# pangenome/impg

Measured on AMD Instinct MI355X. Metric: projected ranges/sec, 1M-PAF 100k-BED -x depth 3; CPU coitrees baseline, higher is better.
Workload: dtype int32

## Files before the change

### impg_amd/csrc/capi.cpp

```cpp
#include <sys/stat.h>
#include <unistd.h>

#include <atomic>
#include <cerrno>
#include <functional>
#include <thread>
#include <chrono>
#include <cmath>
#include <cstdlib>
#include <memory>
#include <new>

#include "engine.hpp"
#include "partition.hpp"
#include "refine.hpp"

namespace impg {
thread_local std::string g_error;
void set_error(const std::string &msg) { g_error = msg; }
void render_paf(const impg_gpu_results &res, const impg_gpu_index &ix, const char *const *range_names,
                const impg_gpu_params_t &p, int32_t merge_distance, bool bedpe, std::vector<std::string> &parts);
void render_bed(const impg_gpu_results &res, const impg_gpu_index &ix, const char *const *range_names,
                const impg_gpu_params_t &p, int32_t merge_distance, std::vector<std::string> &parts);
char *join_parts(std::vector<std::string> &parts, size_t *len);
void render_fasta(const impg_gpu_results &res, const impg_gpu_index &ix, const impg_gpu_params_t &p, int32_t merge_distance, bool reverse_complement,
                  std::vector<std::string> &parts);
}

using namespace impg;


namespace impg {
static void engine_options(impg_gpu_index &ix, Engine *e) {
  const Options &o = e->opt = ix.opt;
  e->walk_allowed = o.walk_kernel != 0 && !getenv("IMPG_NO_WALK");
  e->walk_bfs = o.walk_kernel == 2;
  e->wide_emit = WideEmit{(uint32_t)o.wide_emit_cap, (uint32_t)o.wide_emit_bins, o.lookup_stats != 0};
  e->coop_count = CoopCount{(uint32_t)o.lookup_coop_span, o.lookup_coop != 0};
  e->seg_stats = ix.seg_stats;
  e->proj_stats = ix.proj_stats;
  e->place_block_levels = &ix.place_block_levels;
  e->upd_stats = ix.upd_stats;
  e->dfs_stats = ix.dfs_stats;
  e->lk_stats = ix.lk_stats;
}
static Engine *take_or_create(impg_gpu_index &ix) {
  Engine *e = nullptr;
  if (!ix.eng_free.empty()) { e = ix.eng_free.back(); ix.eng_free.pop_back(); }
  else if ((int)ix.engines.size() < ix.max_engines) {
    ix.engines.emplace_back(new Engine(ix.device));
    e = ix.engines.back().get();
  } else return nullptr;
  engine_options(ix, e);
  return e;
}
EngineLease::EngineLease(impg_gpu_index &ix_) : ix(ix_) {
  std::unique_lock<std::mutex> lk(ix.eng_m);
  while (!(e = take_or_create(ix))) ix.eng_cv.wait(lk);
}
Engine *try_lease_engine(impg_gpu_index &ix) {
  std::unique_lock<std::mutex> lk(ix.eng_m);
  return take_or_create(ix);
}
void return_engine(impg_gpu_index &ix, Engine *e) {
  e->remote = nullptr;
  e->masked = false;
  e->subset_on = false;
  std::lock_guard<std::mutex> lk(ix.eng_m);
  ix.eng_free.push_back(e);
  ix.eng_cv.notify_one();
}
EngineLease::~EngineLease() { return_engine(ix, e); }
}

namespace impg {

void require_device(int device) {
  int n = 0;
  hipError_t e = hipGetDeviceCount(&n);
  if (e != hipSuccess || n <= 0)
    throw Error{IMPG_E_HIP, "no HIP device available (libimpg_gpu has no CPU fallback)"};
  if (device < 0 || device >= n) throw Error{IMPG_E_INVALID, "device ordinal out of range"};
}

std::unique_ptr<impg_gpu_index> make_index(const impg_gpu_record_t *records, size_t n_records, const uint32_t *ops,
                                           size_t n_ops, const int64_t *seq_len, uint32_t n_seq, int bidirectional,
                                           int order_policy, int device, uint32_t shard, uint32_t n_shards,
                                           const HostSeqIndex *seq, const std::vector<uint64_t> *file_first,
                                           const uint32_t *owner) {
  if ((!records && n_records) || (!ops && n_ops) || (!seq_len && n_seq)) throw Error{IMPG_E_INVALID, "null input array"};
  require_device(device);
  auto ix = std::make_unique<impg_gpu_index>();
  ix->device = device;
  if (seq) ix->seq = *seq;
  if (file_first) {
    if (file_first->size() < 2 || file_first->front() != 0 || file_first->back() != n_records ||
        !std::is_sorted(file_first->begin(), file_first->end()))
      throw Error{IMPG_E_INVALID, "file boundaries must start at 0, end at n_records and be ascending"};
    ix->file_first = *file_first;
  }
  build_index(*ix, records, n_records, ops, n_ops, seq_len, n_seq, bidirectional != 0, order_policy, shard, n_shards, owner);
  { EngineLease warm(*ix); }
  return ix;
}

}

namespace impg {
void assemble_results(Engine &E, const impg_gpu_range_t *h_ranges, uint32_t n, const impg_gpu_params_t &p,
                      std::vector<std::unique_ptr<LevelBufs>> &levels, DevBuf &self_dev, impg_gpu_results &res, uint64_t max_rows,
                      hipEvent_t kernels_done, const std::function<void()> &on_kernels_done) {
  hipStream_t s = E.stream;
  res.ranges.assign(h_ranges, h_ranges + n);
  res.has_cigar = p.store_cigar != 0;
  RowPlan pl;
  plan_rows(E, n, p, levels, self_dev, false, pl);
  const size_t nr = pl.n_rows;
  if (nr > max_rows && n > 1) throw SplitBatch{};
  DevBuf rows, clen, coff, cpool;
  for (DevBuf *b : {&rows, &clen, &coff, &cpool}) b->pool = &E.level_pool;
  rows.reserve(std::max<size_t>(nr * sizeof(impg_gpu_interval_t), 256));
  if (res.has_cigar) clen.reserve(std::max<size_t>(nr * 4, 256));
  scatter_rows(E, levels, pl, RowSinks{rows.as<impg_gpu_interval_t>(), nullptr, nullptr, nullptr, nullptr,
                                       res.has_cigar ? clen.as<uint32_t>() : nullptr});
// ... 440 lines not shown
  IMPG_CATCH
}

int impg_gpu_index_load(const char *path, int device, impg_gpu_index_t **out) {
  IMPG_TRY
  if (!path || !out) throw Error{IMPG_E_INVALID, "null argument"};
  require_device(device);
  auto ix = std::make_unique<impg_gpu_index>();
  ix->device = device;
  load_index(*ix, path);
  { EngineLease warm(*ix); }
  *out = ix.release();
  return IMPG_OK;
  IMPG_CATCH
}

void impg_gpu_index_destroy(impg_gpu_index_t *ix) { delete ix; }

uint32_t impg_gpu_num_seqs(const impg_gpu_index_t *ix) { return (uint32_t)ix->seq.lens.size(); }
const char *impg_gpu_seq_name(const impg_gpu_index_t *ix, uint32_t id) {
  return id < ix->seq.names.size() ? ix->seq.names[id].c_str() : nullptr;
}
int64_t impg_gpu_seq_len(const impg_gpu_index_t *ix, uint32_t id) { return id < ix->seq.lens.size() ? ix->seq.lens[id] : -1; }
int64_t impg_gpu_seq_id(const impg_gpu_index_t *ix, const char *name) {
  auto it = ix->seq.name_to_id.find(name);
  return it == ix->seq.name_to_id.end() ? -1 : (int64_t)it->second;
}
size_t impg_gpu_num_targets(const impg_gpu_index_t *ix) { return ix->n_targets; }
size_t impg_gpu_target_ids(const impg_gpu_index_t *ix, uint32_t *out, size_t cap) {
  size_t k = 0;
  for (uint32_t s = 0; s + 1 < ix->h_tgt_off.size(); s++)
    if (ix->h_tgt_off[s + 1] != ix->h_tgt_off[s]) {
      if (out && k < cap) out[k] = s;
      k++;
    }
  return k;
}
size_t impg_gpu_num_entries(const impg_gpu_index_t *ix) { return ix->n_entries; }
size_t impg_gpu_num_records(const impg_gpu_index_t *ix) { return ix->n_records; }
size_t impg_gpu_device_bytes(const impg_gpu_index_t *ix) { return ix->device_bytes; }
int impg_gpu_index_approximate(const impg_gpu_index_t *ix) {
  return ix->tp_mode ? 1 : 0;
}

uint64_t impg_gpu_host_pool_trim(uint64_t keep_bytes) { return (uint64_t)impg::pinned_trim((size_t)keep_bytes); }

static_assert(option_row("walk_members")->hi == WALK_MAX_MEMBERS && option_row("wide_emit_cap")->hi == WIDE_CAP && option_row("wide_emit_bins")->hi == WIDE_BINS && option_row("lookup_coop_span")->hi == LOOKUP_COOP_CAP,
              "the option table's limits are the kernels' capacities");

int impg_gpu_set_option(impg_gpu_index_t *ix, const char *key, int64_t value) {
  IMPG_TRY
  if (!ix || !key) throw Error{IMPG_E_INVALID, "null argument"};
  const OptionRow *row = option_row(key);
  if (!row) throw Error{IMPG_E_INVALID, std::string("unknown option ") + key};
  if (!strcmp(key, "sequence_ingest_piece_bytes") && value % 16) throw Error{IMPG_E_INVALID, row->refusal};
  if (!option_store(ix->opt, *row, value)) throw Error{IMPG_E_INVALID, row->refusal};
  if (row->member || !value) return IMPG_OK;
  if (!strcmp(key, "prewarm_result_bytes")) {
    size_t cap = 0;
    void *b = pinned_take((size_t)value, cap);
    pinned_give(b, cap);
  } else if (!ix->shard && !ix->cluster) {
    IMPG_HIP(hipSetDevice(ix->device));
    EngineLease lease(*ix);
    lease->reserve_walk_slabs(*ix, value >= 2);
  }
  return IMPG_OK;
  IMPG_CATCH
}
const char *impg_gpu_option_key(size_t i) { return i < N_OPTIONS ? OPTION_TABLE[i].key : nullptr; }

struct CounterRow { const char *key; const std::atomic<uint64_t> &(*at)(const impg_gpu_index &); bool over_ranks; };
#define CTR(key, member) {key, [](const impg_gpu_index &ix) -> const std::atomic<uint64_t> & { return ix.member; }, false}
#define CTR_RANKS(key, member) {key, [](const impg_gpu_index &ix) -> const std::atomic<uint64_t> & { return ix.member; }, true}
static const CounterRow COUNTER_TABLE[] = {
    CTR("walk_launches", walk_launches), CTR("walk_fallbacks", walk_fallbacks), CTR("walk_members", walk_last_members), CTR("walk_overflow", walk_last_overflow),
    CTR("small_batches", small_batches),
    CTR("dfs_rounds", dfs_stats[0]), CTR("visited_compactions", dfs_stats[1]),
    CTR("segment_sliced_levels", seg_stats[0]), CTR("segment_retries", seg_stats[1]), CTR("segment_library_levels", seg_stats[2]),
    CTR("project_lane_levels", proj_stats[PROJ_ARM_LANE]), CTR("project_staged_levels", proj_stats[PROJ_ARM_STAGED]),
    CTR("project_staged_rows_levels", proj_stats[PROJ_ARM_STAGED_ROWS]), CTR("project_entries_slots_levels", proj_stats[PROJ_ARM_ENTRIES_SLOTS]),
    CTR("project_entries_qs_levels", proj_stats[PROJ_ARM_ENTRIES_QS]), CTR("project_entries_rows_levels", proj_stats[PROJ_ARM_ENTRIES_ROWS]),
    CTR("project_entries_ident_levels", proj_stats[PROJ_ARM_ENTRIES_IDENT]), CTR("project_tp_levels", proj_stats[PROJ_ARM_TP]),
    CTR("place_offsets_block_levels", place_block_levels),
    CTR("update_lane_groups", upd_stats[UPD_LANE]), CTR("update_mid_groups", upd_stats[UPD_MID]), CTR("update_wave_tiny_groups", upd_stats[UPD_WAVE_TINY]),
    CTR("update_wave_small_groups", upd_stats[UPD_WAVE_SMALL]), CTR("update_wave_large_groups", upd_stats[UPD_WAVE_LARGE]),
    CTR("update_inplace_groups", upd_stats[UPD_INPLACE]), CTR("update_tiled_sort_groups", upd_stats[UPD_TILED_SORT]),
    CTR("update_lane_spill_groups", upd_stats[UPD_LANE_SPILL]),
    CTR("lookup_wide_windows", lk_stats[LK_WIDE]), CTR("lookup_wide_single", lk_stats[LK_SINGLE]), CTR("lookup_wide_grouped", lk_stats[LK_GROUPED]),
    CTR("lookup_wide_group_passes", lk_stats[LK_GROUP_PASSES]), CTR("lookup_wide_overflow", lk_stats[LK_OVERFLOW]),
    CTR("lookup_coop_waves", lk_stats[LK_COOP]), CTR("lookup_lane_waves_mixed", lk_stats[LK_MIXED]), CTR("lookup_lane_waves_span", lk_stats[LK_SPAN]),
    CTR("refine_passes", refine_stats[REFINE_PASSES]), CTR("refine_candidates", refine_stats[REFINE_CANDIDATES]),
    CTR("refine_parts", refine_stats[REFINE_PARTS]), CTR("refine_rows_to_host", refine_stats[REFINE_ROWS_TO_HOST]),
    CTR("refine_longest_group", refine_stats[REFINE_LONGEST_GROUP]),
    CTR("bed_rows", bed_stats[BED_ROWS]), CTR("bed_gap_roots", bed_stats[BED_GAP_ROOTS]), CTR("bed_runs", bed_stats[BED_RUNS]),
    CTR("bed_text_pieces", bed_stats[BED_TEXT_PIECES]), CTR("bed_text_bytes", bed_stats[BED_TEXT_BYTES]),
    CTR("bedpe_rows", bedpe_stats[BEDPE_ROWS]), CTR("bedpe_runs", bedpe_stats[BEDPE_RUNS]),
    CTR("bedpe_joins_contiguous", bedpe_stats[BEDPE_JOINS_CONTIGUOUS]), CTR("bedpe_joins_gap", bedpe_stats[BEDPE_JOINS_GAP]),
    CTR("bedpe_fused_ops", bedpe_stats[BEDPE_FUSED_OPS]), CTR("bedpe_summary_ops", bedpe_stats[BEDPE_SUMMARY_OPS]),
    CTR("bedpe_text_pieces", bedpe_stats[BEDPE_TEXT_PIECES]), CTR("bedpe_text_bytes", bedpe_stats[BEDPE_TEXT_BYTES]),
    CTR("paf_rows", paf_stats[PAF_ROWS]), CTR("paf_runs", paf_stats[PAF_RUNS]),
    CTR("paf_joins_contiguous", paf_stats[PAF_JOINS_CONTIGUOUS]), CTR("paf_joins_gap", paf_stats[PAF_JOINS_GAP]),
    CTR("paf_ops_read", paf_stats[PAF_OPS_READ]), CTR("paf_ops_printed", paf_stats[PAF_OPS_PRINTED]),
    CTR("paf_through_rows", paf_stats[PAF_THROUGH_ROWS]), CTR("paf_text_pieces", paf_stats[PAF_TEXT_PIECES]),
    CTR("paf_text_bytes", paf_stats[PAF_TEXT_BYTES]),
    CTR("fasta_rows", fasta_stats[FASTA_ROWS]), CTR("fasta_records", fasta_stats[FASTA_RECORDS]),
    CTR("fasta_text_pieces", fasta_stats[FASTA_TEXT_PIECES]), CTR("fasta_text_bytes", fasta_stats[FASTA_TEXT_BYTES]),
    CTR("fasta_store_bytes", fasta_stats[FASTA_STORE_BYTES]), CTR("fasta_store_packed", fasta_stats[FASTA_STORE_PACKED]),
    CTR("fasta_store_exception_runs", fasta_stats[FASTA_STORE_EXCEPTION_RUNS]),
    CTR("sequence_ingest_pieces", ingest_stats[0]), CTR("sequence_ingest_text_bytes", ingest_stats[1]), CTR("sequence_ingest_bases", ingest_stats[2]),
    CTR("sequence_ingest_inflated_blocks", ingest_stats[3]), CTR("sequence_ingest_dropped_sequences", ingest_stats[4]),
    CTR_RANKS("build_device", build_stats[BUILD_DEVICE]), CTR_RANKS("tokenized_device", build_stats[BUILD_TOKENIZED_DEVICE]),
    CTR_RANKS("build_batches", build_stats[BUILD_BATCHES]),
};
#undef CTR
#undef CTR_RANKS
constexpr size_t N_COUNTERS = sizeof(COUNTER_TABLE) / sizeof(COUNTER_TABLE[0]);

int impg_gpu_get_counter(const impg_gpu_index_t *ix, const char *key, int64_t *value_out) {
  IMPG_TRY
  if (!ix || !key || !value_out) throw Error{IMPG_E_INVALID, "null argument"};
  for (const CounterRow &c : COUNTER_TABLE)
    if (!strcmp(c.key, key)) {
      uint64_t v = 0;
      if (c.over_ranks) for_each_rank(*ix, [&](const impg_gpu_index &r) { v += c.at(r).load(); });
      else v = c.at(*ix).load();
      *value_out = (int64_t)v;
      return IMPG_OK;
    }
  throw Error{IMPG_E_INVALID, std::string("unknown counter ") + key};
  IMPG_CATCH
}
const char *impg_gpu_counter_key(size_t i) { return i < N_COUNTERS ? COUNTER_TABLE[i].key : nullptr; }

int impg_gpu_visit_rank(uint32_t n, int order_policy, uint32_t *rank_out) {
  IMPG_TRY
  if (!rank_out && n) throw Error{IMPG_E_INVALID, "null argument"};
  if (order_policy == IMPG_ORDER_COITREES) coitrees_visit_rank(n, rank_out);
  else if (order_policy == IMPG_ORDER_SORTED) for (uint32_t i = 0; i < n; i++) rank_out[i] = i;
  else throw Error{IMPG_E_INVALID, "bad order policy"};
  return IMPG_OK;
  IMPG_CATCH
}

}
namespace impg {
void apply_mask(Engine &E, const impg_gpu_index &ix, const impg_gpu_mask_t *m, const impg_gpu_params_t &p) {
  if (!m) return;
  if (!p.transitive) throw Error{IMPG_E_INVALID, "masked_regions belong to the transitive queries"};
  const uint32_t n_seq = ix.view.n_seq;
  if (m->n_seqs && (!m->seq_id || !m->sequence_length || !m->range_off)) throw Error{IMPG_E_INVALID, "null mask array"};
  const uint64_t total = m->n_seqs ? m->range_off[m->n_seqs] : 0;
  if (total >= 0xFFFFFFF0ull) throw Error{IMPG_E_UNSUPPORTED, "mask exceeds 2^32 ranges"};
  if (total && !m->ranges) throw Error{IMPG_E_INVALID, "null mask array"};
  std::vector<uint32_t> off(n_seq + 1, 0);
  std::vector<int32_t> init_len(n_seq, 0), touch_len(n_seq, 0);
  bool has_empty = false;
  if (p.multi_impg) for (uint32_t s = 0; s < n_seq; s++) touch_len[s] = (int32_t)std::min<int64_t>(std::max<int64_t>(ix.seq.lens[s], 0), INT32_MAX);
  for (uint32_t i = 0; i < m->n_seqs; i++) {
    const uint32_t s = m->seq_id[i];
    if (s >= n_seq) throw Error{IMPG_E_INVALID, "mask names an unknown sequence id"};
    if (i && s <= m->seq_id[i - 1]) throw Error{IMPG_E_INVALID, "mask sequence ids must be strictly ascending"};
    if (m->range_off[i + 1] < m->range_off[i]) throw Error{IMPG_E_INVALID, "mask offsets must not decrease"};
    off[s + 1] = (uint32_t)(m->range_off[i + 1] - m->range_off[i]);
    init_len[s] = touch_len[s] = m->sequence_length[i];
    for (uint64_t k = m->range_off[i]; k < m->range_off[i + 1]; k++) {
      const int32_t a = m->ranges[2 * k], b = m->ranges[2 * k + 1];
// ... 841 lines not shown
```

### impg_amd/csrc/engine.cpp

```cpp
#include <cmath>
#include <cstdio>
#include <cstdlib>
#include <memory>

#include "engine.hpp"

namespace impg {

namespace {
inline unsigned bits_for(uint64_t n) {
  unsigned b = 0;
  while ((1ull << b) < n) b++;
  return b;
}
}

Engine::Engine(int device) {
  IMPG_HIP(hipSetDevice(device));
  IMPG_HIP(hipStreamCreateWithFlags(&stream, hipStreamNonBlocking));
  for (DevBuf *b : {&ord_offsets, &ord_rows}) b->pool = &level_pool;
  win_se.pool = &level_pool;
  counters.reserve(128);
  acc_slots.reserve(COUNT_BYTES);
  act_slots.reserve(COUNT_BYTES);
// ... 490 lines not shown
    }
    L.slice_pool.reserve(std::max<size_t>(L.slice_total * 4, 256));
    launch_slice_write(v, pair_entry.as<uint32_t>(), h, sl, L.n_pairs, L.slice_pos.as<uint32_t>(), L.slice_pool.as<uint32_t>(), stream);
  } else {
    L.slice_total = 0;
  }
  timed.push_back({e0, e1, 0});
  timed.push_back({e1, e2, 1});
  if (st) {
    st->pairs += P;
    st->frontier_ranges += n_fr;
    if (P) st->project_launches += 1;
  }
  return P;
}

void Engine::post_expand(const FrontierRec *fr, uint32_t n_fr, LevelBufs &L, const uint32_t *d_pair_off, uint32_t *tie_idx,
                         const uint32_t *tie_rank, SliceArrays sl) {
  HitArrays h{L.qid.as<uint32_t>(), L.coords.as<int4>()};
  if (subset_on)
    launch_subset_filter(fr, L.pair_range.as<uint32_t>(), L.n_pairs, h.qid, subset_keep.as<uint8_t>(), cur_ranges, stream);
  if (multi && L.n_pairs) {
    const size_t b = std::max<size_t>((size_t)L.n_pairs * 4, 256);
    m_dest.reserve(b); m_qid.reserve(b); m_coords.reserve(4 * b); m_pe.reserve(b);
    launch_sort5(fr, n_fr, d_pair_off, L.n_pairs, h, tie_idx, tie_rank, m_dest.as<uint32_t>(), stream);
    HitArrays h2{m_qid.as<uint32_t>(), m_coords.as<int4>()};
    SliceArrays sl2{nullptr, nullptr, nullptr, nullptr};
    if (sl.a) {
      m_sa.reserve(b); m_sn.reserve(b); m_so.reserve(b); m_sr.reserve(b);
      sl2 = SliceArrays{m_sa.as<uint32_t>(), m_sn.as<uint32_t>(), m_so.as<int32_t>(), m_sr.as<int32_t>()};
    }
    launch_permute_slots(m_dest.as<uint32_t>(), L.n_pairs, h, h2, tie_idx, m_pe.as<uint32_t>(), sl, sl2, stream);
    L.qid.swap(m_qid); L.coords.swap(m_coords);
    if (tie_idx == pair_entry.as<uint32_t>()) pair_entry.swap(m_pe);
    if (sl.a) { L.sl_a.swap(m_sa); L.sl_n.swap(m_sn); L.sl_off.swap(m_so); L.sl_rem.swap(m_sr); }
  }
}

void Engine::ordered_level(const FrontierRec *fr, uint32_t n_fr, LevelBufs &L, bool counts_by_range, uint64_t P) {
  const uint64_t total = scan(counts_by_range ? cnt.as<uint32_t>() : ord_cnt.as<uint32_t>(), L.slot_ref.as<uint32_t>(), n_fr);
  if (total != P) throw Error{IMPG_E_INVALID, "internal: a level's slot counts disagree between its two orders"};
  L.lvbase.reserve(std::max<size_t>((size_t)ord_n * 4, 256));
  launch_ord_level_bases(fr, n_fr, L.slot_ref.as<uint32_t>(), (uint32_t)P, ord_n, ord_acc.as<uint32_t>(), L.lvbase.as<uint32_t>(), stream);
}
void Engine::ordered_offsets() {
  if (ord_offsets_done) return;
  ord_offsets.reserve(((size_t)ord_n + 1) * 4);
  ord_total = scan(ord_acc.as<uint32_t>(), ord_offsets.as<uint32_t>(), ord_n + 1u);
  if (ord_total >= 0xFFFFFFF0ull) { if (split_ok) throw SplitBatch{}; throw Error{IMPG_E_UNSUPPORTED, "more than 2^32 result rows in one chunk: use smaller chunks (chunk_ranges)"}; }
  ord_rows.reserve(std::max<size_t>(ord_total * sizeof(impg_gpu_interval_t), 256));
  ord_offsets_done = true;
}
void Engine::ordered_finish(std::vector<std::unique_ptr<LevelBufs>> &levels) {
  hipEvent_t p0 = event(), p1 = event();
  IMPG_HIP(hipEventRecord(p0, stream));
  ordered_offsets();
  launch_ord_self_rows(ord_self, ord_ranges, ord_n, ord_offsets.as<uint32_t>(), ord_rows.as<impg_gpu_interval_t>(), stream);
  for (auto &Lp : levels) {
    LevelBufs &L = *Lp;
    if (L.placed || !L.n_pairs) continue;
    L.run_start.reserve(std::max<size_t>((size_t)L.n_frontier * 4, 256));
    launch_ord_run_heads(L.pair_range.as<uint32_t>(), L.n_pairs, L.run_start.as<uint32_t>(), stream);
    HitArrays h{L.qid.as<uint32_t>(), L.coords.as<int4>()};
    launch_ord_level_rows(L.frontier.as<FrontierRec>(), L.pair_range.as<uint32_t>(), L.n_pairs, h, L.run_start.as<uint32_t>(), L.slot_ref.as<uint32_t>(),
                          ord_offsets.as<uint32_t>(), L.lvbase.as<uint32_t>(), ord_min_len, ord_rows.as<impg_gpu_interval_t>(), stream);
    L.placed = true;
  }
  IMPG_HIP(hipEventRecord(p1, stream));
  IMPG_HIP(hipStreamSynchronize(stream));
  float ms = 0;
  IMPG_HIP(hipEventElapsedTime(&ms, p0, p1));
  ms_place = ms;
}

HopResult Engine::hop(const DeviceIndexView &v, const FrontierRec *fr, uint32_t n_fr, bool transitive, LevelBufs &L,
                      impg_gpu_stats_t *st, bool need_hits, bool need_rows, bool alive) {
  if (remote) return remote->hop(*this, v, fr, n_fr, transitive, L, st, need_hits, need_rows, alive);
  if (!alive) { L.n_pairs = 0; return HopResult{0, true}; }
  if (!n_fr) { L.n_pairs = 0; return HopResult{0, false}; }
  return HopResult{expand(v, fr, n_fr, transitive, L, st), false};
}

uint32_t Engine::update(const DeviceIndexView &v, const FrontierRec *fr, LevelBufs &L, uint32_t n_queries,
                        const impg_gpu_params_t &p, DevBuf &next_frontier) {
  hipEvent_t e0 = event(), e1 = event();
  IMPG_HIP(hipEventRecord(e0, stream));
  const uint32_t P = L.n_pairs;
  uint32_t n_next = 0;
  HitArrays h{L.qid.as<uint32_t>(), L.coords.as<int4>()};
  if (P) {
    const uint32_t P_slots = P;
    const bool want_flags = opt.filter_covered != 0;
    svals.reserve((size_t)P * 8);
    uint32_t seg_active = 0, seg_groups = 0;
    uint32_t *sg_run_start = nullptr, *sg_run_end = nullptr, *sg_q = nullptr, *sg_bins = nullptr;
    uint32_t seg_parts = opt.segment_groups && !want_flags && !multi && seg_group_fits(v.n_seq) && L.n_frontier > 0 ? seg_group_parts(P, n_queries, v.n_seq) : 0u;
    if (opt.segment_parts && seg_parts) {
      seg_parts = std::max(1u, std::min((uint32_t)opt.segment_parts, 4096u));
      while (seg_parts > 1 && ((uint64_t)n_queries * seg_parts >= (1ull << 31) || seg_group_bins_bytes(n_queries, v.n_seq, seg_parts) > (1ull << 30))) seg_parts >>= 1;
    }
    bool by_segments = seg_parts != 0;
    if (by_segments) {
      const uint32_t n_fr = L.n_frontier;
      seg_run.reserve(std::max<size_t>((size_t)n_fr * 8, 256));
      seg_q.reserve(std::max<size_t>((size_t)n_queries * 24 + 256, 512));
      sg_run_start = seg_run.as<uint32_t>(); sg_run_end = sg_run_start + n_fr;
      sg_q = seg_q.as<uint32_t>();
      uint32_t *qfirst = sg_q, *qlast = qfirst + n_queries, *qact = qlast + n_queries, *qdst = qact + n_queries, *qgrp = qdst + n_queries,
               *gdst = qgrp + n_queries, *unsorted = gdst + n_queries;
      const bool own_offsets = !remote && !store_cigar && L.n_frontier == expand_n_fr;
      launch_seg_bounds(fr, n_fr, n_queries, L.pair_range.as<uint32_t>(), P, sg_run_start, sg_run_end, qfirst, qlast, unsorted, stream,
                        own_offsets && last_by_place ? lo_perm.as<uint32_t>() : nullptr, own_offsets ? pair_off.as<uint32_t>() : nullptr,
                        own_offsets ? cnt.as<uint32_t>() : nullptr);
      for (int attempt = 0; attempt < 2 && by_segments; attempt++) {
        const size_t bb = seg_group_bins_bytes(n_queries, v.n_seq, seg_parts);
        sg_bins = nullptr;
        if (seg_parts > 1 || bb <= (512ull << 20)) { seg_bins.reserve(std::max<size_t>(bb, 256)); sg_bins = seg_bins.as<uint32_t>(); }
        if (seg_parts > 1) seg_tot.reserve(std::max<size_t>(seg_group_bins_bytes(n_queries, v.n_seq, 1), 256));
        launch_seg_group(true, fr, qfirst, qlast, sg_run_start, sg_run_end, h, n_queries, v.n_seq, qact, qdst, qgrp, gdst, nullptr, nullptr, nullptr, sg_bins,
                         stream, seg_parts, seg_tot.as<uint32_t>());
        uint64_t ta = 0, tg = 0;
        uint32_t bad[2] = {0, 0};
        scan2(qact, qdst, qgrp, gdst, n_queries, ta, tg, unsorted, bad, 2);
        seg_active = (uint32_t)ta;
        if (bad[0]) by_segments = false;
        else if (bad[1]) {
          const uint32_t again = seg_parts == 1 && attempt == 0 ? seg_group_parts(P, n_queries, v.n_seq, bad[1]) : 0u;
          if (again > 1) { seg_parts = again; IMPG_HIP(hipMemsetAsync(unsorted, 0, 8, stream)); if (seg_stats) seg_stats[1]++; }
          else by_segments = false;
        } else { seg_groups = (uint32_t)tg; break; }
      }
      if (by_segments && seg_parts > 1 && seg_stats) seg_stats[0]++;
    }
    if (!by_segments) {
      if (seg_stats) seg_stats[2]++;
      keys.reserve((size_t)P * 8); skeys.reserve((size_t)P * 8); vals.reserve((size_t)P * 8);
      IMPG_HIP(hipMemsetAsync(act_slots.p, 0, COUNT_BYTES, stream));
      launch_update_keys(fr, L.pair_range.as<uint32_t>(), P, h, keys.as<unsigned long long>(), vals.as<unsigned long long>(),
                         act_slots.as<unsigned long long>(), stream);
      size_t tb = sort_u64v_scratch_bytes(P);
      sort_tmp.reserve(tb);
      const unsigned sbits = std::max(1u, bits_for(v.n_seq)), qbits = std::max(1u, bits_for(n_queries));
      launch_sort_u64v(sort_tmp.p, tb, keys.as<unsigned long long>(), skeys.as<unsigned long long>(), vals.as<unsigned long long>(),
                       svals.as<unsigned long long>(), P, stream, sbits, 0);
      launch_sort_u64v(sort_tmp.p, tb, skeys.as<unsigned long long>(), keys.as<unsigned long long>(), svals.as<unsigned long long>(),
                       vals.as<unsigned long long>(), P, stream, std::min(64u, 32 + qbits + 1), 32);
      keys.swap(skeys);
      vals.swap(svals);
    }
    const uint32_t P = by_segments ? seg_active : P_slots;
    uint32_t n_groups;
    if (by_segments) n_groups = seg_groups;
    else if (want_flags) {
      head.reserve((size_t)P * 4); gid.reserve((size_t)P * 4);
      launch_group_heads(skeys.as<unsigned long long>(), P, head.as<uint32_t>(), stream);
      n_groups = (uint32_t)scan(head.as<uint32_t>(), gid.as<uint32_t>(), P);
    } else {
      const uint32_t nt = group_tiles(P);
      head.reserve((size_t)nt * 4); gid.reserve((size_t)nt * 4);
      launch_group_count(skeys.as<unsigned long long>(), P, head.as<uint32_t>(), stream);
      n_groups = (uint32_t)scan(head.as<uint32_t>(), gid.as<uint32_t>(), nt);
    }
    if (n_groups) {
      auto vt = std::make_unique<VisitedStore>(&table_pool);
      vt->keys.reserve((size_t)n_groups * 8);
      gstart.reserve((size_t)n_groups * 4);
      if (by_segments) {
        uint32_t *qfirst = sg_q, *qlast = qfirst + n_queries, *qact = qlast + n_queries, *qdst = qact + n_queries, *qgrp = qdst + n_queries,
                 *gdst = qgrp + n_queries;
        launch_seg_group(false, fr, qfirst, qlast, sg_run_start, sg_run_end, h, n_queries, v.n_seq, qact, qdst, qgrp, gdst, gstart.as<uint32_t>(),
                         vt->keys.as<unsigned long long>(), svals.as<unsigned long long>(), sg_bins, stream, seg_parts, seg_tot.as<uint32_t>());
      } else if (want_flags)
        launch_group_scatter(skeys.as<unsigned long long>(), P, head.as<uint32_t>(), gid.as<uint32_t>(), gstart.as<uint32_t>(),
                             vt->keys.as<unsigned long long>(), stream);
      else
        launch_group_fill(skeys.as<unsigned long long>(), P, gid.as<uint32_t>(), gstart.as<uint32_t>(), vt->keys.as<unsigned long long>(), stream);
      const uint32_t n_active = by_segments ? seg_active : (uint32_t)read_slots(act_slots);
      glen.reserve((size_t)n_groups * 4); old_src.reserve((size_t)n_groups * 8);
      cap.reserve((size_t)n_groups * 4); pcap.reserve((size_t)n_groups * 4);
      VisitedTables tabs = tables_view();
      launch_group_prepare(tabs, vt->keys.as<unsigned long long>(), gstart.as<uint32_t>(), n_groups, n_active,
                           glen.as<uint32_t>(), old_src.as<const int2 *>(), cap.as<uint32_t>(),
                           pcap.as<uint32_t>(), stream);
      if (getenv("IMPG_DEBUG_GROUPS")) {
        std::vector<uint32_t> hc(n_groups), hp(n_groups), hl(n_groups);
        IMPG_HIP(hipStreamSynchronize(stream));
        IMPG_HIP(hipMemcpy(hc.data(), cap.p, (size_t)n_groups * 4, hipMemcpyDeviceToHost));
        IMPG_HIP(hipMemcpy(hp.data(), pcap.p, (size_t)n_groups * 4, hipMemcpyDeviceToHost));
        IMPG_HIP(hipMemcpy(hl.data(), glen.p, (size_t)n_groups * 4, hipMemcpyDeviceToHost));
        uint64_t b[8] = {0}, hits[8] = {0};
        const uint32_t edge[8] = {16, 64, 512, 1024, 2048, 4096, 16384, 0xFFFFFFFFu};
        uint32_t mx = 0, mxl = 0;
        for (uint32_t g2 = 0; g2 < n_groups; g2++) {
          int k = 0;
          while (hc[g2] > edge[k]) k++;
          b[k]++; hits[k] += hl[g2];
          mx = std::max(mx, hc[g2]); mxl = std::max(mxl, hl[g2]);
        }
        {
          uint64_t bc[21] = {0}, bh[21] = {0};
          for (uint32_t g2 = 0; g2 < n_groups; g2++) { bc[std::min(hc[g2], 20u)]++; bh[std::min(hl[g2], 20u)]++; }
          fprintf(stderr, "[groups] by cap 1..20+:");
          for (int k2 = 1; k2 <= 20; k2++) fprintf(stderr, " %llu", (unsigned long long)bc[k2]);
          fprintf(stderr, "\n[groups] by hits 1..20+:");
          for (int k2 = 1; k2 <= 20; k2++) fprintf(stderr, " %llu", (unsigned long long)bh[k2]);
          fprintf(stderr, "\n");
        }
        fprintf(stderr, "[groups] n=%u P=%u maxcap=%u maxhits=%u | cap<=16:%llu(%llu) 64:%llu(%llu) 512:%llu(%llu) 1k:%llu(%llu) 2k:%llu(%llu) 4k:%llu(%llu) 16k:%llu(%llu) more:%llu(%llu)\n",
                n_groups, P, mx, mxl, (unsigned long long)b[0], (unsigned long long)hits[0], (unsigned long long)b[1], (unsigned long long)hits[1],
                (unsigned long long)b[2], (unsigned long long)hits[2], (unsigned long long)b[3], (unsigned long long)hits[3],
                (unsigned long long)b[4], (unsigned long long)hits[4], (unsigned long long)b[5], (unsigned long long)hits[5],
                (unsigned long long)b[6], (unsigned long long)hits[6], (unsigned long long)b[7], (unsigned long long)hits[7]);
      }
      const unsigned long long *replay_vals = svals.as<unsigned long long>();
      const bool filter = opt.filter_covered == 1 || (opt.filter_covered == 2 && tables.size() >= 2 && (uint64_t)n_active >= 8ull * n_groups);
      if (filter && n_active) {
        uint32_t *keep = keys.as<uint32_t>(), *kpos = keep + P;
        launch_covered_flags(svals.as<unsigned long long>(), head.as<uint32_t>(), gid.as<uint32_t>(), vt->keys.as<unsigned long long>(),
                             old_src.as<const int2 *>(), cap.as<uint32_t>(), glen.as<uint32_t>(), masked ? mask_touch_len.as<int32_t>() : v.seq_len,
                             n_active, keep, stream);
        const uint32_t n_kept = (uint32_t)scan(keep, kpos, n_active);
        launch_covered_compact(svals.as<unsigned long long>(), keep, kpos, n_active, vals.as<unsigned long long>(), n_kept, n_groups,
                               gstart.as<uint32_t>(), glen.as<uint32_t>(), cap.as<uint32_t>(), pcap.as<uint32_t>(), stream);
        replay_vals = vals.as<unsigned long long>();
        covered_dropped += n_active - n_kept;
      }
      vt->off.reserve((size_t)n_groups * 4);
      poff.reserve((size_t)n_groups * 4);
      uint64_t cap_total = 0, pcap_total = 0;
      big_list.reserve((size_t)n_groups * 12);
      uint32_t *d_nbig = (uint32_t *)(counters.as<uint64_t>() + 8);
      uint32_t h_lists[VU_LIST_WORDS] = {0};
      launch_big_groups(cap.as<uint32_t>(), pcap.as<uint32_t>(), n_groups, big_list.as<uint32_t>(), d_nbig, stream);
      scan2(cap.as<uint32_t>(), vt->off.as<uint32_t>(), pcap.as<uint32_t>(), poff.as<uint32_t>(), n_groups, cap_total, pcap_total, d_nbig, h_lists,
            VU_LIST_WORDS);
      if (cap_total >= 0xFFFFFFF0ull || pcap_total >= 0xFFFFFFF0ull)
        { if (split_ok) throw SplitBatch{}; throw Error{IMPG_E_UNSUPPORTED, "visited sets exceed 2^32 ranges"}; }
      vt->ranges.reserve(std::max<size_t>(cap_total * 8, 256));
      vt->len.reserve((size_t)n_groups * 4);
      pieces.reserve(std::max<size_t>(pcap_total * 8, 256));
      n_pieces.reserve((size_t)n_groups * 4);
      foff.reserve((size_t)n_groups * 4);
      launch_visited_update(replay_vals, masked ? mask_touch_len.as<int32_t>() : v.seq_len, vt->keys.as<unsigned long long>(),
                            gstart.as<uint32_t>(), glen.as<uint32_t>(), old_src.as<const int2 *>(),
                            vt->off.as<uint32_t>(), poff.as<uint32_t>(), n_groups, p.min_transitive_len,
                            p.min_distance_between_ranges, vt->ranges.as<int2>(), vt->len.as<uint32_t>(),
                            pieces.as<int2>(), n_pieces.as<uint32_t>(), cap.as<uint32_t>(), pcap.as<uint32_t>(), big_list.as<uint32_t>(),
                            d_nbig, opt.update_stats && upd_stats, stream, h_lists);
      uint64_t nn = scan(n_pieces.as<uint32_t>(), foff.as<uint32_t>(), n_groups);
      if (opt.update_stats && upd_stats && n_groups) {
        IMPG_HIP(hipMemcpyAsync(h_counters, counters.as<uint64_t>() + 8, VU_NBIG_WORDS * 4, hipMemcpyDeviceToHost, stream));
        IMPG_HIP(hipStreamSynchronize(stream));
        const uint32_t *w = reinterpret_cast<const uint32_t *>(h_counters), *reach = w + VU_REACH_BASE;
        upd_stats[UPD_LANE] += n_groups - (w[0] + w[1] + w[2] + w[6]);
        upd_stats[UPD_MID] += w[6];
        upd_stats[UPD_WAVE_TINY] += w[2];
        upd_stats[UPD_WAVE_SMALL] += w[0];
        upd_stats[UPD_WAVE_LARGE] += w[1];
        upd_stats[UPD_INPLACE] += reach[VU_REACH_INPLACE];
        upd_stats[UPD_TILED_SORT] += reach[VU_REACH_TILED_SORT];
        upd_stats[UPD_LANE_SPILL] += reach[VU_REACH_LANE_SPILL];
      }
      if (nn >= 0xFFFFFFF0ull) { if (split_ok) throw SplitBatch{}; throw Error{IMPG_E_UNSUPPORTED, "frontier exceeds 2^32 ranges"}; }
      n_next = (uint32_t)nn;
      next_frontier.reserve(std::max<size_t>((size_t)n_next * sizeof(FrontierRec), 256));
      const bool keys_too = !remote && opt.locality_min && n_next >= opt.locality_min;
      if (keys_too) { lo_key.reserve((size_t)n_next * 4); lo_idx.reserve((size_t)n_next * 4); }
      launch_frontier_emit(vt->keys.as<unsigned long long>(), poff.as<uint32_t>(), n_pieces.as<uint32_t>(),
                           foff.as<uint32_t>(), n_groups, pieces.as<int2>(), next_frontier.as<FrontierRec>(), stream,
                           keys_too ? &v : nullptr, lo_key.as<uint32_t>(), lib_sort_selected() ? lo_idx.as<uint32_t>() : nullptr);
      keys_for = keys_too ? next_frontier.p : nullptr;
      keys_n = n_next;
      vt->n_groups = n_groups;
      index_table(*vt);
      tables.push_back(std::move(vt));
      if (tables.size() + 2 >= (size_t)MAX_VISITED_TABLES) compact_tables();
    }
  }
  IMPG_HIP(hipEventRecord(e1, stream));
  timed.push_back({e0, e1, 2});
  return n_next;
}

void Engine::index_table(VisitedStore &t) {
  t.qoff.reserve(((size_t)table_queries + 1) * 4);
  launch_table_qoff(t.keys.as<unsigned long long>(), t.n_groups, table_queries, t.qoff.as<uint32_t>(), stream);
}

VisitedTables Engine::tables_view() const {
  VisitedTables t;
  memset(&t, 0, sizeof t);
  t.n_tables = (uint32_t)tables.size();
  for (size_t i = 0; i < tables.size(); i++) {
    t.t[i].keys = tables[i]->keys.as<unsigned long long>();
    t.t[i].off = tables[i]->off.as<uint32_t>();
    t.t[i].len = tables[i]->len.as<uint32_t>();
    t.t[i].ranges = tables[i]->ranges.as<int2>();
    t.t[i].qoff = tables[i]->qoff.as<uint32_t>();
    t.t[i].n_groups = tables[i]->n_groups;
  }
  if (masked) {
    t.mask_off = mask_off.as<uint32_t>();
    t.mask_ranges = mask_ranges.as<int2>();
  }
  return t;
}

uint32_t Engine::begin_transitive(const DeviceIndexView &v, const impg_gpu_range_t *d_ranges, uint32_t n,
                                  const impg_gpu_params_t &p, FrontierRec *d_self, DevBuf &frontier_out) {
  tables.clear();
  auto t = std::make_unique<VisitedStore>(&table_pool);
  t->keys.reserve((size_t)n * 8); t->off.reserve((size_t)n * 4); t->len.reserve((size_t)n * 4);
  t->ranges.reserve((size_t)n * 8);
  t->n_groups = n;
  head.reserve((size_t)n * 4); gid.reserve((size_t)n * 4);
  launch_visited_init(d_ranges, n, v.seq_len, v.n_seq, p.min_transitive_len, t->keys.as<unsigned long long>(),
                      t->off.as<uint32_t>(), t->len.as<uint32_t>(), t->ranges.as<int2>(), d_self, head.as<uint32_t>(), stream);
  uint32_t n_fr = (uint32_t)scan(head.as<uint32_t>(), gid.as<uint32_t>(), n);
  frontier_out.reserve(std::max<size_t>((size_t)n_fr * sizeof(FrontierRec), 256));
  launch_compact_frontier(d_self, head.as<uint32_t>(), gid.as<uint32_t>(), n, frontier_out.as<FrontierRec>(), stream);
  table_queries = n;
  index_table(*t);
  tables.push_back(std::move(t));
  return n_fr;
}

uint32_t Engine::begin_transitive_masked(const DeviceIndexView &v, const impg_gpu_range_t *d_ranges, uint32_t n,
                                         const impg_gpu_params_t &p, DevBuf &self, DevBuf &frontier_out) {
  tables.clear();
  auto t = std::make_unique<VisitedStore>(&table_pool);
  t->keys.reserve((size_t)n * 8); t->off.reserve((size_t)n * 4 + 4); t->len.reserve((size_t)n * 4);
  t->n_groups = n;
  cap.reserve((size_t)n * 4);
  launch_mask_caps(d_ranges, n, mask_off.as<uint32_t>(), v.n_seq, cap.as<uint32_t>(), stream);
  const uint64_t total = scan(cap.as<uint32_t>(), t->off.as<uint32_t>(), n);
  if (total >= 0xFFFFFFF0ull) { if (split_ok) throw SplitBatch{}; throw Error{IMPG_E_UNSUPPORTED, "visited sets exceed 2^32 ranges"}; }
  t->ranges.reserve(std::max<size_t>(total * 8, 256));
  pieces.reserve(std::max<size_t>(total * 8, 256));
  n_pieces.reserve((size_t)n * 4); head.reserve((size_t)n * 4); gid.reserve((size_t)n * 4);
  self_off.reserve((size_t)n * 4 + 4);
  launch_visited_init_masked(d_ranges, n, mask_init_len.as<int32_t>(), v.n_seq, mask_off.as<uint32_t>(), mask_ranges.as<int2>(),
                             p.min_transitive_len, t->off.as<uint32_t>(), t->keys.as<unsigned long long>(),
                             t->len.as<uint32_t>(), t->ranges.as<int2>(), pieces.as<int2>(), n_pieces.as<uint32_t>(),
                             head.as<uint32_t>(), stream);
  n_self = scan(n_pieces.as<uint32_t>(), self_off.as<uint32_t>(), n);
  const uint32_t n_fr = (uint32_t)scan(head.as<uint32_t>(), gid.as<uint32_t>(), n);
  self.reserve(std::max<size_t>((size_t)n_self * sizeof(FrontierRec), 256));
  frontier_out.reserve(std::max<size_t>((size_t)n_fr * sizeof(FrontierRec), 256));
  launch_masked_self_emit(d_ranges, n, t->off.as<uint32_t>(), n_pieces.as<uint32_t>(), self_off.as<uint32_t>(),
                          gid.as<uint32_t>(), p.min_transitive_len, pieces.as<int2>(), self.as<FrontierRec>(),
                          frontier_out.as<FrontierRec>(), stream);
  table_queries = n;
  index_table(*t);
  tables.push_back(std::move(t));
  return n_fr;
}

void Engine::check_params(const impg_gpu_params_t &p) {
  if (p.transitive && p.max_depth > 65535) throw Error{IMPG_E_INVALID, "max_depth is a u16 in the reference"};
// ... 36 lines not shown
  hipEvent_t t0 = event(), t1 = event();
  IMPG_HIP(hipEventRecord(t0, stream));
  if (st) memset(st, 0, sizeof *st);
  const bool transitive = p.transitive != 0;
  if (!keep && !self_out && walk_applicable(ix, n, p)) {
    ev_next = 0;
    if (run_walk(ix, d_ranges, n, p, d_count, d_cksum, st, nullptr)) return;
    if (d_count) IMPG_HIP(hipMemsetAsync(d_count, 0, (size_t)n * 8, stream));
    if (d_cksum) IMPG_HIP(hipMemsetAsync(d_cksum, 0, (size_t)n * 8, stream));
    ev_next = 0;
    timed.clear();
    IMPG_HIP(hipMemsetAsync(counters.p, 0, 64, stream));
    IMPG_HIP(hipMemsetAsync(acc_slots.p, 0, COUNT_BYTES, stream));
    t0 = event(); t1 = event();
    IMPG_HIP(hipEventRecord(t0, stream));
    if (st) memset(st, 0, sizeof *st);
  }
  if (transitive && (p.dfs || multi)) {
    ev_next = 0;
    run_dfs(ix, spec);
    return;
  }

  DevBuf *cur = &frontier_a, *nxt = &frontier_b;
  uint32_t n_fr = 0;
  cur->reserve(std::max<size_t>((size_t)n * sizeof(FrontierRec), 256));
  if (!n) {
  } else if (!transitive) {
    launch_ranges_to_frontier(d_ranges, n, cur->as<FrontierRec>(), (uint32_t *)(counters.as<uint64_t>() + 5), stream);
    n_fr = n;
  } else {
    DevBuf &self = self_out ? *self_out : self_scratch;
    self.reserve(std::max<size_t>((size_t)n * sizeof(FrontierRec), 256));
    n_fr = masked ? begin_transitive_masked(v, d_ranges, n, p, self, *cur)
                  : begin_transitive(v, d_ranges, n, p, self.as<FrontierRec>(), *cur);
    ord_self = self.as<FrontierRec>();
  }
  if (ordered_rows) {
    if (!keep || masked || multi || store_cigar || remote) throw Error{IMPG_E_INVALID, "internal: ordered rows are placed for plain and BFS batches of one GPU"};
    ord_n = n;
    ord_ranges = d_ranges;
    if (!transitive) ord_self = nullptr;
    ord_min_len = transitive ? p.min_output_length : -1;
    ord_offsets_done = false;
    ord_total = 0;
    ms_place = 0;
    ord_acc.reserve(((size_t)n + 1) * 4);
    IMPG_HIP(hipMemsetAsync(ord_acc.p, 0, ((size_t)n + 1) * 4, stream));
    launch_ord_self_count(ord_self, d_ranges, n, ord_acc.as<uint32_t>(), stream);
  }

  uint32_t depth = 0;
  for (;;) {
    const bool alive = n_fr > 0 && (!transitive || p.max_depth == 0 || depth < p.max_depth);
    const bool last = !transitive || (p.max_depth > 0 && depth + 1 >= p.max_depth);
    std::unique_ptr<LevelBufs> own;
    LevelBufs *L = &level_scratch;
    if (keep) {
      own = std::make_unique<LevelBufs>(remote_rows ? remote_rows->pool : &level_pool);
      L = own.get();
    }
    const bool want_stats = d_count || d_cksum;
    const bool owners_keep = keep && remote && remote_rows && last;
    if (owners_keep) remote_rows->level = depth;
    fuse_final = opt.fuse_final_level && last && (!keep || spec.keep_any_order || ordered_rows) && !remote;
    if (want_stats && (uint64_t)n_fr > 8192ull * n) fuse_final = false;
    fuse_need_ranges = want_stats || subset_on || keep != nullptr;
    fuse_range_places = keep != nullptr && !want_stats && !subset_on;
    if (ordered_rows) fuse_need_ranges = fuse_range_places = false;
    const HopResult hr = hop(v, cur->as<FrontierRec>(), alive ? n_fr : 0, transitive, *L, st,
                             !owners_keep && (keep || want_stats || !last), !owners_keep && (keep || d_cksum), alive);
    fuse_final = false;
    if (hr.all_dead) break;
    uint32_t n_next = 0;
    if (alive) {
      L->n_frontier = n_fr;
      if (want_stats) {
        HitArrays h{L->qid.as<uint32_t>(), L->coords.as<int4>()};
        rstat.reserve(std::max<size_t>((size_t)n_fr * 16, 256));
        launch_hit_stats(cur->as<FrontierRec>(), n_fr, L->pair_range.as<uint32_t>(), L->n_pairs, h,
                         transitive ? p.min_output_length : -1, false, rstat.as<unsigned long long>(), d_count, d_cksum, stream);
      }
      if (st) st->levels += 1;
      if (!last) n_next = update(v, cur->as<FrontierRec>(), *L, n, p, *nxt);
      if (keep && !owners_keep) {
        if (L->placed) {
        } else if (last_range_places && !remote) {
          L->frontier.adopt(win_se);
        } else {
          L->frontier.reserve(std::max<size_t>((size_t)n_fr * sizeof(FrontierRec), 256));
          IMPG_HIP(hipMemcpyAsync(L->frontier.p, cur->p, (size_t)n_fr * sizeof(FrontierRec), hipMemcpyDeviceToDevice, stream));
        }
        keep->push_back(std::move(own));
      }
    }
    if (last) break;
    std::swap(cur, nxt);
    n_fr = n_next;
    depth += 1;
  }
  if (ordered_rows) ordered_finish(*keep);
  finish_run(st, t0, t1);
}

void Engine::finish_run(impg_gpu_stats_t *st, hipEvent_t t0, hipEvent_t t1) {
  IMPG_HIP(hipEventRecord(t1, stream));
  IMPG_HIP(hipStreamSynchronize(stream));
  uint64_t hc[6];
  IMPG_HIP(hipMemcpy(hc, counters.p, 48, hipMemcpyDeviceToHost));
  if (hc[5]) throw Error{IMPG_E_INVALID, "query range must satisfy start < end"};
  if (hc[2] & 2) throw Error{IMPG_E_INVALID, "Projection resulted in negative query coordinates"};
  if (hc[2] & 4) throw Error{IMPG_E_INVALID, "CIGAR operation length exceeds 29 bits"};
  if (hc[2]) throw Error{IMPG_E_INVALID, "an alignment hit by the query has no CIGAR (missing cg:Z tag)"};
  hc[1] = read_slots(acc_slots);
  if (st) {
    st->projected = hc[1];
    float ms = 0;
    IMPG_HIP(hipEventElapsedTime(&ms, t0, t1));
    st->ms_total = ms;
    for (auto &te : timed) {
      IMPG_HIP(hipEventElapsedTime(&ms, te.a, te.b));
      if (te.kind == 0) st->ms_lookup += ms;
      else if (te.kind == 1) st->ms_project += ms;
      else st->ms_update += ms;
    }
  }
  last_projected = hc[1];
}

void Engine::compact_tables() {
  if (tables.size() < 2) return;
  uint64_t G = 0;
  for (auto &t : tables) G += t->n_groups;
  if (G >= 0xFFFFFFF0ull) throw Error{IMPG_E_UNSUPPORTED, "visited tables exceed 2^32 groups"};
  const uint32_t g = (uint32_t)G;
  VisitedTables tv = tables_view();
  d_ckey.reserve((size_t)g * 8); d_ckey2.reserve((size_t)g * 8); d_src.reserve((size_t)g * 8); d_src2.reserve((size_t)g * 8);
  uint32_t off = 0;
  for (size_t t = 0; t < tables.size(); t++) {
    launch_compact_fill(tables[t]->keys.as<unsigned long long>(), tables[t]->n_groups, (uint32_t)t,
                        d_ckey.as<unsigned long long>() + off, d_src.as<unsigned long long>() + off, stream);
    off += tables[t]->n_groups;
  }
  size_t tb = sort_u64v_scratch_bytes(g);
  sort_tmp.reserve(tb);
  launch_sort_u64v(sort_tmp.p, tb, d_ckey.as<unsigned long long>(), d_ckey2.as<unsigned long long>(),
                   d_src.as<unsigned long long>(), d_src2.as<unsigned long long>(), g, stream);
  d_flag2.reserve((size_t)g * 4); d_pos2.reserve((size_t)g * 4);
  launch_compact_last(d_ckey2.as<unsigned long long>(), g, d_flag2.as<uint32_t>(), stream);
  const uint32_t g2 = (uint32_t)scan(d_flag2.as<uint32_t>(), d_pos2.as<uint32_t>(), g);
  auto nt = std::make_unique<VisitedStore>(&table_pool);
  nt->keys.reserve((size_t)g2 * 8); nt->off.reserve((size_t)g2 * 4); nt->len.reserve((size_t)g2 * 4);
  launch_compact_select(tv, d_ckey2.as<unsigned long long>(), d_src2.as<unsigned long long>(), g, d_flag2.as<uint32_t>(),
                        d_pos2.as<uint32_t>(), nt->keys.as<unsigned long long>(), d_src.as<unsigned long long>(),
                        nt->len.as<uint32_t>(), stream);
  const uint64_t total = scan(nt->len.as<uint32_t>(), nt->off.as<uint32_t>(), g2);
  if (total >= 0xFFFFFFF0ull) throw Error{IMPG_E_UNSUPPORTED, "visited sets exceed 2^32 ranges"};
  nt->ranges.reserve(std::max<size_t>(total * 8, 256));
  launch_compact_copy(tv, d_src.as<unsigned long long>(), nt->off.as<uint32_t>(), nt->len.as<uint32_t>(), g2,
                      nt->ranges.as<int2>(), stream);
  nt->n_groups = g2;
  index_table(*nt);
  IMPG_HIP(hipStreamSynchronize(stream));
  tables.clear();
  tables.push_back(std::move(nt));
  if (dfs_stats) dfs_stats[1]++;
}
// ... 129 lines not shown
```

### impg_amd/csrc/engine.hpp

```cpp
#pragma once
#include <atomic>
#include <functional>
#include <memory>
#include <string>
#include <vector>

#include "kernels.hpp"

namespace impg {

struct LevelBufs {
  DevBuf frontier, pair_range, qid, coords;
  DevBuf sl_a, sl_n, sl_off, sl_rem, slice_pos, slice_pool;
  uint64_t slice_total = 0;
  uint32_t n_frontier = 0, n_pairs = 0;
  DevBuf slot_ref, lvbase, run_start;
  bool qs_interleaved = false;
  bool placed = false;
  LevelBufs() = default;
  explicit LevelBufs(BufPool *pool) {
    for (DevBuf *b : {&frontier, &pair_range, &qid, &coords, &sl_a, &sl_n, &sl_off, &sl_rem, &slice_pos, &slice_pool, &slot_ref, &lvbase, &run_start}) b->pool = pool;
  }
};
struct VisitedStore {
// ... 37 lines not shown
  RunSpec(const impg_gpu_range_t *d_ranges_, uint32_t n_, const impg_gpu_params_t &p_) : d_ranges(d_ranges_), n(n_), p(p_) {}
};

struct Engine {
  BufPool table_pool;
  BufPool level_pool;
  hipStream_t stream = nullptr;
  DevBuf counters;
  DevBuf acc_slots, act_slots;
  uint64_t *h_slots = nullptr;
  uint64_t read_slots(DevBuf &b);
  uint64_t *h_counters = nullptr;
  std::vector<hipEvent_t> ev_pool;
  size_t ev_next = 0;
  struct Timed { hipEvent_t a, b; int kind; };
  std::vector<Timed> timed;
  DevBuf big_list;
  DevBuf cnt, win, pair_off, pair_entry, scan_tmp, scan_tmp2, keys, skeys, vals, svals, sort_tmp, head, gid, gstart, glen, old_src,
      cap, pcap, poff, pieces, n_pieces, foff, frontier_a, frontier_b, self_scratch, ranges_dev, stat_count,
      stat_cksum, stage_off;
  LevelBufs level_scratch;
  std::vector<std::unique_ptr<VisitedStore>> tables;
  uint32_t table_queries = 0;
  void index_table(VisitedStore &t);
  uint64_t last_projected = 0;
  Options opt;
  bool split_ok = false;
  double min_identity = __builtin_nan("");
  bool store_cigar = false;
  bool multi = false;
  bool free_slot_order = false;
  bool fuse_final = false, fuse_need_ranges = false, fuse_range_places = false;
  bool last_range_places = false;
  DevBuf ord_acc, ord_offsets, ord_rows, ord_dest, ord_vpos, ord_cnt;
  uint64_t ord_total = 0;
  bool ord_offsets_done = false;
  uint32_t ord_n = 0;
  int32_t ord_min_len = -1;
  const FrontierRec *ord_self = nullptr;
  const impg_gpu_range_t *ord_ranges = nullptr;
  void ordered_level(const FrontierRec *fr, uint32_t n_fr, LevelBufs &L, bool counts_by_range, uint64_t P);
  void ordered_offsets();
  void ordered_finish(std::vector<std::unique_ptr<LevelBufs>> &levels);
  float ms_place = 0;
  DevBuf ent_work, ent_alloc;
  DevBuf win_se, tile_first;
  DevBuf place_local, place_sum, place_base;
  uint64_t covered_dropped = 0;
  DevBuf m_dest, m_qid, m_coords, m_pe, m_sa, m_sn, m_so, m_sr;
  DevBuf wide_n, wide_list;
  WideEmit wide_emit;
  CoopCount coop_count;
  std::atomic<uint64_t> *lk_stats = nullptr;
  void count_wide_paths(const DeviceIndexView &v, uint32_t n);
  DevBuf lo_key, lo_key2, lo_idx, lo_perm, lo_cnt, lo_off, lo_offp, slot_of;
  const uint32_t *stage_perm = nullptr;
  uint32_t stage_n = 0;

  explicit Engine(int device);
  ~Engine();
  hipEvent_t event();
  uint64_t read_counter(int k);
  uint64_t scan(const uint32_t *in, uint32_t *out, uint32_t n, const uint32_t *d_extra = nullptr, uint32_t *h_extra = nullptr, uint32_t n_extra = 0);
  void scan2(const uint32_t *in_a, uint32_t *out_a, const uint32_t *in_b, uint32_t *out_b, uint32_t n, uint64_t &total_a, uint64_t &total_b,
             const uint32_t *d_extra = nullptr, uint32_t *h_extra = nullptr, uint32_t n_extra = 0);
  struct RecordBlocks { const uint32_t *d_bounds; uint32_t n_blocks; };
  const uint32_t *lookup_order(const DeviceIndexView &v, const FrontierRec *fr, uint32_t n_fr, const RecordBlocks *blocks = nullptr);
  void projection_offsets(const uint32_t *d_perm, uint32_t n_fr, const uint32_t *d_cnt, uint64_t P, const uint32_t *&d_offp,
                          ProjList &pl);
  DevBuf proj_range, proj_entry;
  uint64_t expand(const DeviceIndexView &v, const FrontierRec *fr, uint32_t n_fr, bool transitive, LevelBufs &L,
                  impg_gpu_stats_t *st, bool raw = false, const RecordBlocks *blocks = nullptr);
  const void *keys_for = nullptr;
  uint32_t keys_n = 0;
  uint32_t expand_n_fr = 0;
  bool last_by_place = false;
  void post_expand(const FrontierRec *fr, uint32_t n_fr, LevelBufs &L, const uint32_t *d_pair_off, uint32_t *tie_idx,
                   const uint32_t *tie_rank, SliceArrays sl);
  Expander *remote = nullptr;
  const RunModes &modes() const { return run_modes; }
  HopResult hop(const DeviceIndexView &v, const FrontierRec *fr, uint32_t n_fr, bool transitive, LevelBufs &L,
                impg_gpu_stats_t *st, bool need_hits, bool need_rows, bool alive);
  uint32_t update(const DeviceIndexView &v, const FrontierRec *fr, LevelBufs &L, uint32_t n_queries,
                  const impg_gpu_params_t &p, DevBuf &next_frontier);
  VisitedTables tables_view() const;
  void compact_tables();
  DevBuf dk_a, dk_b, ds_a, ds_b, de_a, de_b, dd_a, dd_b, d_flag2, d_pos2, d_popdepth, d_popsel, d_perm, d_perm2, d_k32, d_k32b,
      d_src, d_src2, d_ckey, d_ckey2;
  void run_dfs(const impg_gpu_index &ix, const RunSpec &spec);
  void finish_run(impg_gpu_stats_t *st, hipEvent_t t0, hipEvent_t t1);
  static void check_params(const impg_gpu_params_t &p);
  uint32_t begin_transitive(const DeviceIndexView &v, const impg_gpu_range_t *d_ranges, uint32_t n,
                            const impg_gpu_params_t &p, FrontierRec *d_self, DevBuf &frontier_out);
  DevBuf subset_keep;
  bool subset_on = false;
  const impg_gpu_range_t *cur_ranges = nullptr;
  bool masked = false;
  DevBuf mask_off, mask_ranges, mask_init_len, mask_touch_len;
  bool mask_has_empty = false;
  uint64_t mask_ranges_total = 0, mask_lists = 0;
  DevBuf self_off;
  uint64_t n_self = 0;
  uint32_t begin_transitive_masked(const DeviceIndexView &v, const impg_gpu_range_t *d_ranges, uint32_t n,
                                   const impg_gpu_params_t &p, DevBuf &self, DevBuf &frontier_out);
  float stage_ms[3] = {0, 0, 0};
  uint64_t stage_launches = 0;
  DevBuf stage_next;
  uint32_t stage_next_n = 0, stage_queries = 0;
  void run(const impg_gpu_index &ix, const RunSpec &spec);
  static constexpr uint32_t SMALL_RANGES = 64, SMALL_PAIRS = 1u << 18;
  bool run_small(const impg_gpu_index &ix, const impg_gpu_range_t *h_ranges, uint32_t n, const impg_gpu_params_t &p,
                 impg_gpu_results &res);
  struct WalkRows {
    DevBuf rows, base, cap, n_rows;
    std::vector<uint32_t> h_n_rows;
    std::vector<unsigned long long> h_base;
  };
  bool walk_allowed = true, walk_bfs = false;
  bool walk_applicable(const impg_gpu_index &ix, uint32_t n, const impg_gpu_params_t &p) const;
  static void walk_caps(bool wide, WalkArgs &a);
  static uint64_t walk_workgroups(const impg_gpu_index &ix, bool wide);
  void reserve_walk_slabs(const impg_gpu_index &ix, bool dfs_too);
  bool run_walk(const impg_gpu_index &ix, const impg_gpu_range_t *d_ranges, uint32_t n, const impg_gpu_params_t &p,
                unsigned long long *d_count, unsigned long long *d_cksum, impg_gpu_stats_t *st, WalkRows *rows, uint32_t *h_n_rows = nullptr);
  DevBuf walk_slabs, walk_ctr, walk_ctl;
  DevBuf rstat;
  DevBuf seg_run, seg_q, seg_bins, seg_tot;
  std::atomic<uint64_t> *seg_stats = nullptr;
  std::atomic<uint64_t> *proj_stats = nullptr;
  std::atomic<uint64_t> *upd_stats = nullptr;
  std::atomic<uint64_t> *dfs_stats = nullptr;
  std::atomic<uint64_t> *place_block_levels = nullptr;
  void count_arm(int arm) { if (proj_stats && arm >= 0 && arm < PROJ_ARMS) proj_stats[arm]++; }
  uint32_t walk_group_size(const impg_gpu_index &ix, uint32_t n, const impg_gpu_params_t &p) const;
  char *small_in = nullptr;
  char *small_out = nullptr;
  void *small_out_dev = nullptr;
  size_t small_out_cap = 0;

 private:
  RunModes run_modes;
};

void build_index(impg_gpu_index &ix, const impg_gpu_record_t *records, size_t n_records, const uint32_t *cigar_ops,
                 size_t n_ops, const int64_t *seq_len, uint32_t n_seq, bool bidirectional, int order_policy,
                 uint32_t shard, uint32_t n_shards, const uint32_t *owner, const TpInput *tp = nullptr,
                 const EntryPlan *plan = nullptr);

struct EngineLease {
  impg_gpu_index &ix;
  Engine *e = nullptr;
  explicit EngineLease(impg_gpu_index &ix);
  ~EngineLease();
  EngineLease(const EngineLease &) = delete;
  Engine &operator*() { return *e; }
  Engine *operator->() { return e; }
};

#define IMPG_TRY try {
#define IMPG_CATCH                                          \
  }                                                         \
  catch (const impg::Error &e) {                            \
    impg::set_error(e.msg);                                 \
    return e.code;                                          \
  }                                                         \
  catch (const std::bad_alloc &) {                          \
    impg::set_error("host out of memory");                  \
    return IMPG_E_OOM;                                      \
  }                                                         \
  catch (const std::exception &e) {                         \
    impg::set_error(std::string("internal: ") + e.what());  \
    return IMPG_E_INVALID;                                  \
  }
void require_device(int device);
std::unique_ptr<impg_gpu_index> make_index(const impg_gpu_record_t *records, size_t n_records, const uint32_t *ops,
                                           size_t n_ops, const int64_t *seq_len, uint32_t n_seq, int bidirectional,
                                           int order_policy, int device, uint32_t shard, uint32_t n_shards,
                                           const HostSeqIndex *seq, const std::vector<uint64_t> *file_first,
                                           const uint32_t *owner);
void assemble_results(Engine &E, const impg_gpu_range_t *h_ranges, uint32_t n, const impg_gpu_params_t &p,
                      std::vector<std::unique_ptr<LevelBufs>> &levels, DevBuf &self_dev, impg_gpu_results &res,
                      uint64_t max_rows = ~0ull, hipEvent_t kernels_done = nullptr,
                      const std::function<void()> &on_kernels_done = nullptr);
const impg_gpu_range_t *upload_ranges(DevBuf &dst, const impg_gpu_range_t *ranges, size_t n, const hipStream_t *async_on);
inline void add_stats(impg_gpu_stats_t &tot, const impg_gpu_stats_t &st) {
  tot.projected += st.projected; tot.pairs += st.pairs; tot.frontier_ranges += st.frontier_ranges;
  tot.levels = std::max(tot.levels, st.levels);
  tot.ms_total += st.ms_total; tot.ms_lookup += st.ms_lookup; tot.ms_project += st.ms_project; tot.ms_update += st.ms_update;
  tot.project_launches += st.project_launches;
  tot.ms_exchange += st.ms_exchange;
}
struct StatSinks {
  unsigned long long *count = nullptr, *cksum = nullptr;
  StatSinks(DevBuf &cnt, DevBuf &ck, bool want_count, bool want_cksum, size_t n, const hipStream_t *async_on);
  void aim(RunSpec &rs, size_t b) const { rs.d_count = count ? count + b : nullptr; rs.d_cksum = cksum ? cksum + b : nullptr; }
  void home(uint64_t *per_range_count, uint64_t *per_range_checksum, size_t n) const;
};
inline std::unique_lock<std::mutex> take_turn(std::mutex *gpu_turn) {
  return gpu_turn ? std::unique_lock<std::mutex>(*gpu_turn) : std::unique_lock<std::mutex>();
}
bool run_chunk_rows(const impg_gpu_index &ix, Engine &E, const impg_gpu_range_t *d_ranges, const impg_gpu_range_t *h_ranges, size_t b,
                    size_t e, const impg_gpu_params_t &p, impg_gpu_results &part, std::mutex *gpu_turn = nullptr,
                    uint64_t max_rows = ~0ull, hipEvent_t kernels_done = nullptr,
                    const std::function<void()> &on_kernels_done = nullptr);
enum TextFormat { TEXT_BED = 0, TEXT_BEDPE = 1, TEXT_PAF = 2, TEXT_FASTA = 3, TEXT_FASTA_RC = 4 };
bool run_chunk_bed(const impg_gpu_index &ix, Engine &E, const impg_gpu_range_t *d_ranges, const impg_gpu_range_t *h_ranges,
                   const char *const *range_names, size_t b, size_t e, const impg_gpu_params_t &p, int32_t merge_distance,
                   const std::function<void(const char *, size_t)> &sink, double *seconds3, std::mutex *gpu_turn = nullptr,
                   TextFormat format = TEXT_BED);
struct RowPlan {
  DevBuf flag, pos;
  DevBuf rec_start, rec_dest;
  DevBuf offsets;
  uint64_t n_slots = 0, n_recs = 0;
  uint32_t n_rows = 0, n_self = 0;
// ... 101 lines not shown
```

### impg_amd/csrc/impg_internal.hpp

```cpp
#pragma once
#include <atomic>
#include <chrono>
#include <exception>
#include <functional>
#include <vector>
#include <hip/hip_runtime.h>

#include <algorithm>
#include <condition_variable>
#include <cstdlib>
#include <new>
#include <cstdint>
#include <cstring>
#include <memory>
#include <mutex>
#include <string>
#include <unordered_map>
#include <vector>

#include "../../include/impg_gpu.h"
#include "options.hpp"

namespace impg {

// ... 272 lines not shown
    return off;
  }
  s += name;
  return 0;
}

enum BuildStat { BUILD_DEVICE, BUILD_TOKENIZED_DEVICE, BUILD_BATCHES };
void for_each_rank(const impg_gpu_index &ix, const std::function<void(const impg_gpu_index &)> &f);
enum BedStat { BED_ROWS, BED_GAP_ROOTS, BED_RUNS, BED_TEXT_PIECES, BED_TEXT_BYTES };
enum BedpeStat { BEDPE_ROWS, BEDPE_RUNS, BEDPE_JOINS_CONTIGUOUS, BEDPE_JOINS_GAP, BEDPE_FUSED_OPS, BEDPE_SUMMARY_OPS, BEDPE_TEXT_PIECES, BEDPE_TEXT_BYTES };
enum PafStat { PAF_ROWS, PAF_RUNS, PAF_JOINS_CONTIGUOUS, PAF_JOINS_GAP, PAF_OPS_READ, PAF_OPS_PRINTED, PAF_THROUGH_ROWS, PAF_TEXT_PIECES, PAF_TEXT_BYTES };
size_t bed_merge(impg_gpu_interval_t *iv, size_t n, int32_t merge_distance, bool merge_strands);
void query_axis_merge(std::vector<impg_gpu_interval_t> &rows, int32_t merge_distance, bool merge_strands);

enum FastaStat { FASTA_ROWS, FASTA_RECORDS, FASTA_TEXT_PIECES, FASTA_TEXT_BYTES, FASTA_STORE_BYTES, FASTA_STORE_PACKED, FASTA_STORE_EXCEPTION_RUNS };
struct SeqStore {
  std::vector<std::string> names;
  std::vector<uint64_t> off;
  std::string bases;
  std::unordered_map<std::string, uint32_t> by_name;
  bool device_only = false;
  void add(const std::string &name, const char *b, size_t n);
};
inline const SeqStore &host_copy(const SeqStore &st) {
  if (st.device_only)
    throw Error{IMPG_E_UNSUPPORTED, "the sequences were loaded straight into HBM (impg_gpu_index_load_sequences) and have no host copy: "
                                    "attach them with impg_gpu_index_set_sequences for FASTA text written on the host"};
  return st;
}
constexpr uint32_t SEQ_ABSENT = 0xFFFFFFFFu;
constexpr uint64_t SEQ_NOT_IN_HBM = ~0ull;
constexpr size_t SEQ_PAD = 16;
struct SeqRun { uint32_t start, end; uint8_t byte; };
void seq_exception_runs(const char *bases, size_t n, std::vector<SeqRun> &runs);
struct SeqRef { const char *bases; uint64_t len; };
void fasta_range_text(std::vector<impg_gpu_interval_t> &rows, int32_t merge_distance, bool reverse_complement,
                      const std::function<bool(uint32_t, std::string &, SeqRef &)> &fetch, std::string &text);
void partition_fasta_text(const impg_gpu_partition_row_t *rows, size_t n, const std::function<bool(uint32_t, std::string &, SeqRef &)> &fetch,
                          std::string &text);

struct Engine;
struct ShardCtx;
struct Cluster;

}

struct impg_gpu_index {
  int device = 0;
  hipStream_t stream = nullptr;
  impg::HostSeqIndex seq;
  size_t n_records = 0, n_entries = 0, n_tiles = 0, n_targets = 0;
  std::vector<uint32_t> h_tgt_off;
  std::vector<uint64_t> file_first;
  impg::DevBuf d_seg, d_starts, d_ends, d_ends_t, d_pmax, d_starts_lvl, d_pmax_lvl, d_rank, d_mrank, d_entries, d_ops, d_ext_cp, d_idp, d_seq_len, d_pfx;
  impg::DeviceIndexView view{};
  static constexpr int N_BLOBS = 15;
  impg::DevBuf *blob(int k);
  size_t blob_bytes[N_BLOBS] = {};
  bool multi_file = false;
  bool tp_mode = false;
  void bind_view(uint32_t n_seq, uint32_t sorted_order);
  std::atomic<size_t> device_bytes{0};
  std::mutex idl_m;
  void ensure_identity_lines();
  std::atomic<bool> has_identity_lines{false};
  bool lacks_identity_lines() const {
    return !tp_mode && n_tiles && blob_bytes[14] && !has_identity_lines.load(std::memory_order_acquire);
  }
  std::vector<std::unique_ptr<impg::Engine>> engines;
  std::vector<impg::Engine *> eng_free;
  std::mutex eng_m;
  std::condition_variable eng_cv;
  int max_engines = 4;
  impg::Options opt;
  struct RowsPool : impg::BufPool { RowsPool() { shared = true; } } rows_pool;
  mutable std::atomic<uint64_t> walk_launches{0}, walk_fallbacks{0}, walk_last_members{1}, walk_last_overflow{0};
  mutable std::atomic<uint64_t> small_batches{0};
  mutable std::atomic<uint64_t> dfs_stats[2] = {};
  mutable std::atomic<uint64_t> build_stats[3] = {};
  mutable std::atomic<uint64_t> mask_table_uploads{0}, result_rows_to_host{0};
  mutable std::atomic<uint64_t> seg_stats[3] = {};
  mutable std::atomic<uint64_t> proj_stats[8] = {};
  mutable std::atomic<uint64_t> place_block_levels{0};
  mutable std::atomic<uint64_t> upd_stats[8] = {};
  mutable std::atomic<uint64_t> lk_stats[8] = {};
  mutable std::atomic<uint64_t> refine_stats[5] = {};
  mutable std::atomic<uint64_t> bed_stats[5] = {};
  void bed_stats_reset() const { for (auto &b : bed_stats) b = 0; }
  mutable std::atomic<uint64_t> bedpe_stats[8] = {};
  void bedpe_stats_reset() const { for (auto &b : bedpe_stats) b = 0; }
  mutable std::atomic<uint64_t> paf_stats[9] = {};
  void paf_stats_reset() const { for (auto &b : paf_stats) b = 0; }
  mutable std::atomic<uint64_t> fasta_stats[7] = {};
  mutable std::atomic<uint64_t> ingest_stats[5] = {};
  void fasta_stats_reset() const { for (int k = 0; k < impg::FASTA_STORE_BYTES; k++) fasta_stats[k] = 0; }
  std::shared_ptr<const impg::SeqStore> seq_store;
  std::vector<uint32_t> store_of_id;
  impg::DevBuf d_seq_bases, d_seq_off;
  bool seq_packed = false;
  impg::DevBuf d_seq_run_off, d_seq_runs, d_seq_run_byte, d_seq_blk_off, d_seq_blk;
  void drop_device_sequences();
  impg::ShardCtx *shard = nullptr;
  impg::Cluster *cluster = nullptr;
  impg_gpu_index();
  ~impg_gpu_index();
};

struct impg_gpu_results {
  std::vector<uint64_t> offsets;
  impg::HostArr<impg_gpu_interval_t> intervals;
  std::vector<impg_gpu_range_t> ranges;
  bool has_cigar = false;
  bool approximate = false;
  impg::HostArr<uint64_t> cigar_off;
  impg::HostArr<uint32_t> cigar_ops;
  uint64_t projected = 0;
  double run_s = 0, assemble_s = 0;
};
```

### impg_amd/csrc/kernels.hip

```cpp
#include <hip/hip_runtime.h>

#include <cstring>
#include <type_traits>

#include "device_prims.hpp"
#include "impg_internal.hpp"
#include "kernels.hpp"

namespace impg {

__device__ __forceinline__ unsigned lane_id() { return threadIdx.x & 63u; }
__device__ __forceinline__ unsigned long long lanemask_lt() { return (1ull << lane_id()) - 1ull; }

template <int CTRL, int ROW_MASK>
__device__ __forceinline__ uint32_t dpp_or0(uint32_t x) {
  return (uint32_t)__builtin_amdgcn_update_dpp(0, (int)x, CTRL, ROW_MASK, 0xF, false);
}
__device__ __forceinline__ uint32_t wave_incl_scan(uint32_t x) {
  x += dpp_or0<0x111, 0xF>(x);
  x += dpp_or0<0x112, 0xF>(x);
  x += dpp_or0<0x114, 0xF>(x);
  x += dpp_or0<0x118, 0xF>(x);
  x += dpp_or0<0x142, 0xA>(x);
  x += dpp_or0<0x143, 0xC>(x);
// ... 2953 lines not shown
  bool should_add = true;
  if (mdbr > 0) {
    const uint32_t idx = list_lower_bound(R, len, start);
    if (idx > 0 && abs(start - R.y(idx - 1)) < mdbr) should_add = false;
    if (should_add && idx < len && abs(R.x(idx) - end) < mdbr) should_add = false;
  }
  if (!should_add) return;
  if (start < 0) start = 0;
  if (end > sequence_length) end = sequence_length;
  int32_t current = start;
  const uint32_t pos = list_lower_bound(R, len, start);
  uint32_t i = pos;
  if (i > 0 && R.y(i - 1) > start) i -= 1;
  while (i < len && current < end) {
    const int32_t rx = R.x(i), ry = R.y(i);
    if (rx > end) break;
    if (current < rx) {
      if (abs(rx - current) >= min_transitive_len) emit(current, rx);
    }
    current = max(current, ry);
    i += 1;
  }
  if (current < end) {
    if (abs(end - current) >= min_transitive_len) emit(current, end);
  }
  uint32_t mfrom;
  if (pos > 0 && R.y(pos - 1) >= start) {
    R.y(pos - 1) = max(R.y(pos - 1), end);
    mfrom = pos - 1;
  } else if (pos < len && end >= R.x(pos)) {
    R.x(pos) = min(start, R.x(pos));
    R.y(pos) = max(end, R.y(pos));
    mfrom = pos;
  } else {
    grow();
    for (uint32_t k = len; k > pos; k--) { R.x(k) = R.x(k - 1); R.y(k) = R.y(k - 1); }
    R.x(pos) = start;
    R.y(pos) = end;
    len += 1;
    return;
  }
  uint32_t write = mfrom, read = mfrom + 1;
  while (read < len) {
    if (R.y(write) >= R.x(read)) {
      R.y(write) = max(R.y(write), R.y(read));
    } else {
      write += 1;
      const int32_t tx = R.x(write), ty = R.y(write);
      R.x(write) = R.x(read); R.y(write) = R.y(read);
      R.x(read) = tx; R.y(read) = ty;
    }
    read += 1;
  }
  len = write + 1;
}
template <class L>
__device__ __forceinline__ uint32_t replay_hits(const L &R, uint32_t len, const unsigned long long *__restrict__ svals,
                                                uint32_t st, uint32_t n, int32_t sequence_length,
                                                int32_t min_transitive_len, int32_t mdbr, int2 *__restrict__ P, uint32_t &np) {
  for (uint32_t t = 0; t < n; t++) {
    const unsigned long long iv = svals[st + t];
    replay_one(R, len, (int32_t)(uint32_t)(iv >> 32), (int32_t)(uint32_t)iv, sequence_length, min_transitive_len, mdbr,
               [&](int32_t a, int32_t b) { P[np++] = make_int2(a, b); }, [] {});
  }
  return len;
}
#ifdef IMPG_VU_CLOCKS
constexpr uint32_t VU_CLK_ROWS = 1024;
__device__ unsigned long long g_vu_clk[VU_CLK_ROWS][16];
#define VU_MARK(i) do { asm volatile("s_waitcnt vmcnt(0) lgkmcnt(0)" ::: "memory"); vu_t[i] = __builtin_readcyclecounter(); } while (0)
#else
#define VU_MARK(i) do { } while (0)
#endif
typedef const unsigned long long __attribute__((address_space(1))) *global_list_t;
__device__ __forceinline__ int2 list_range(global_list_t p, uint32_t i) {
  const unsigned long long v = p[i];
  return make_int2((int32_t)(uint32_t)v, (int32_t)(uint32_t)(v >> 32));
}
#ifndef IMPG_VU_WAVES
#define IMPG_VU_WAVES 6
#endif
#pragma clang diagnostic push
#pragma clang diagnostic ignored "-Wpass-failed"
template <uint32_t CAP, bool LISTED>
__global__ __launch_bounds__(64) __attribute__((amdgpu_waves_per_eu(IMPG_VU_WAVES, IMPG_VU_WAVES)))
void visited_update_kernel(const unsigned long long *__restrict__ svals,
                                                            const int32_t *__restrict__ seq_len,
                                                            const unsigned long long *__restrict__ gkey,
                                                            const uint32_t *__restrict__ gstart,
                                                            const uint32_t *__restrict__ glen,
                                                            const unsigned long long *__restrict__ old_src,
                                                            const uint32_t *__restrict__ cap,
                                                            const uint32_t *__restrict__ noff,
                                                            const uint32_t *__restrict__ poff, uint32_t n_groups,
                                                            int32_t min_transitive_len, int32_t mdbr,
                                                            int2 *__restrict__ new_ranges, uint32_t *__restrict__ new_len,
                                                            int2 *__restrict__ pieces, uint32_t *__restrict__ n_pieces,
                                                            const uint32_t *__restrict__ list, const uint32_t *__restrict__ n_list,
                                                            uint32_t *__restrict__ reach) {
  __shared__ int32_t lds_x[CAP * 64], lds_y[CAP * 64];
  const uint32_t n_items = LISTED ? *n_list : n_groups;
  for (uint32_t item0 = blockIdx.x * 64u; item0 < n_items; item0 += gridDim.x * 64u) {
  const uint32_t item = item0 + threadIdx.x;
#ifdef IMPG_VU_CLOCKS
  unsigned long long vu_t[8];
  VU_MARK(0);
#endif
  const bool have = item < n_items;
  const uint32_t g = LISTED ? list[min(item, n_items - 1u)] : item;
  const uint32_t gi = min(g, n_groups - 1u);
  const uint32_t c_ = cap[gi], n_ = glen[gi], st_ = gstart[gi], no = noff[gi], po = poff[gi];
  const global_list_t src_ = (global_list_t)old_src[gi];
  const unsigned long long key = gkey[gi];
  const uint32_t c = have ? c_ : 0u;
  const bool mine = have && (LISTED || c <= VU_TINY_MAX);
  const uint32_t n = mine ? n_ : 0u, st = mine ? st_ : 0u;
  const uint32_t olen = mine ? c - n : 0u;
  int2 *R = new_ranges + no;
  int2 *P = pieces + po;
  VU_MARK(1);
  const int32_t sequence_length = seq_len[(uint32_t)(key & 0xFFFFFFFFull)];
  const unsigned long long *hp = svals + st;
  const uint32_t hl = max(n, 1u) - 1u;
  unsigned long long h0 = hp[0], h1 = hp[min(1u, hl)], h2 = hp[min(2u, hl)], h3 = hp[min(3u, hl)];
  const global_list_t src = olen ? src_ : (global_list_t)(unsigned long long)(uintptr_t)svals;
  const uint32_t sl = max(olen, 1u) - 1u;
  const int2 s0 = list_range(src, 0), s1 = list_range(src, min(1u, sl)), s2 = list_range(src, min(2u, sl)), s3 = list_range(src, min(3u, sl));
  VU_MARK(2);
  uint32_t len = olen, np = 0;
  VU_MARK(3);
  const bool fast = mine;
  const ListInLds A{lds_x + threadIdx.x, lds_y + threadIdx.x};
  if (fast) {
    if (olen > 0) { A.x(0) = s0.x; A.y(0) = s0.y; }
    if (olen > 1) { A.x(1) = s1.x; A.y(1) = s1.y; }
    if (olen > 2) { A.x(2) = s2.x; A.y(2) = s2.y; }
    if (olen > 3) { A.x(3) = s3.x; A.y(3) = s3.y; }
    for (uint32_t i = 4; i < olen; i += 4) {
      const uint32_t l = olen - 1u;
      const int2 r0 = list_range(src, i), r1 = list_range(src, min(i + 1u, l)), r2 = list_range(src, min(i + 2u, l)), r3 = list_range(src, min(i + 3u, l));
      A.x(i) = r0.x; A.y(i) = r0.y;
      if (i + 1u < olen) { A.x(i + 1u) = r1.x; A.y(i + 1u) = r1.y; }
      if (i + 2u < olen) { A.x(i + 2u) = r2.x; A.y(i + 2u) = r2.y; }
      if (i + 3u < olen) { A.x(i + 3u) = r3.x; A.y(i + 3u) = r3.y; }
    }
  }
  VU_MARK(4);
  const uint32_t nf = fast ? n : 0u;
  const uint32_t nmax = wave_max_u32(nf);
  bool spilled = false;
  auto spill = [&]() {
    for (uint32_t k = 0; k < np; k++) P[k] = make_int2(A.x(CAP - 1u - k), A.y(CAP - 1u - k));
    spilled = true;
  };
  auto emit = [&](int32_t a, int32_t b) {
    if (!spilled && len + np >= CAP) spill();
    if (!spilled) { A.x(CAP - 1u - np) = a; A.y(CAP - 1u - np) = b; }
    else P[np] = make_int2(a, b);
    np += 1;
  };
  auto grow = [&]() { if (!spilled && len + np >= CAP) spill(); };
  for (uint32_t t0 = 0; t0 < nmax; t0 += 4u) {
    unsigned long long q0 = 0, q1 = 0, q2 = 0, q3 = 0;
    if (t0 + 4u < nmax && nf) {
      const unsigned long long *hp = svals + st;
      const uint32_t l = nf - 1u;
      q0 = hp[min(t0 + 4u, l)]; q1 = hp[min(t0 + 5u, l)]; q2 = hp[min(t0 + 6u, l)]; q3 = hp[min(t0 + 7u, l)];
    }
#pragma nounroll
    for (uint32_t k = 0; k < 4u; k++) {
      const unsigned long long iv = h0;
      h0 = h1; h1 = h2; h2 = h3;
      if (t0 + k < nf)
        replay_one(A, len, (int32_t)(uint32_t)(iv >> 32), (int32_t)(uint32_t)iv, sequence_length, min_transitive_len, mdbr, emit, grow);
    }
    h0 = q0; h1 = q1; h2 = q2; h3 = q3;
  }
  VU_MARK(5);
  if (fast) for (uint32_t i = 0; i < len; i++) R[i] = make_int2(A.x(i), A.y(i));
  VU_MARK(6);
  if (fast && !spilled) {
    const uint32_t T = CAP - 1u;
    for (uint32_t i = 1; i < np; i++) {
      const int32_t tx = A.x(T - i), ty = A.y(T - i);
      uint32_t j = i;
      while (j > 0 && A.x(T - (j - 1u)) > tx) { A.x(T - j) = A.x(T - (j - 1u)); A.y(T - j) = A.y(T - (j - 1u)); j--; }
      A.x(T - j) = tx; A.y(T - j) = ty;
    }
    if (np) {
      uint32_t w = 0;
      int32_t cx = A.x(T), cy = A.y(T);
      for (uint32_t r = 1; r < np; r++) {
        const int32_t rx = A.x(T - r), ry = A.y(T - r);
        if (cy >= rx) cy = max(cy, ry);
        else { P[w] = make_int2(cx, cy); w += 1; cx = rx; cy = ry; }
      }
      P[w] = make_int2(cx, cy);
      np = w + 1;
    }
  } else if (mine && np > 1 && np <= CAP) {
    const ListInLds S{lds_x + threadIdx.x, lds_y + threadIdx.x};
    for (uint32_t i = 0; i < np; i += 4) {
      const uint32_t l = np - 1u;
      const int2 r0 = P[i], r1 = P[min(i + 1u, l)], r2 = P[min(i + 2u, l)], r3 = P[min(i + 3u, l)];
      S.x(i) = r0.x; S.y(i) = r0.y;
      if (i + 1u < np) { S.x(i + 1u) = r1.x; S.y(i + 1u) = r1.y; }
      if (i + 2u < np) { S.x(i + 2u) = r2.x; S.y(i + 2u) = r2.y; }
      if (i + 3u < np) { S.x(i + 3u) = r3.x; S.y(i + 3u) = r3.y; }
    }
    for (uint32_t i = 1; i < np; i++) {
      const int32_t tx = S.x(i), ty = S.y(i);
      uint32_t j = i;
      while (j > 0 && S.x(j - 1) > tx) { S.x(j) = S.x(j - 1); S.y(j) = S.y(j - 1); j--; }
      S.x(j) = tx; S.y(j) = ty;
    }
    uint32_t w = 0;
    int32_t cx = S.x(0), cy = S.y(0);
    for (uint32_t r = 1; r < np; r++) {
      const int32_t rx = S.x(r), ry = S.y(r);
      if (cy >= rx) cy = max(cy, ry);
      else { P[w] = make_int2(cx, cy); w += 1; cx = rx; cy = ry; }
    }
    P[w] = make_int2(cx, cy);
    np = w + 1;
  } else if (mine) {
    for (uint32_t i = 1; i < np; i++) {
      int2 x = P[i];
      uint32_t j = i;
      while (j > 0 && P[j - 1].x > x.x) { P[j] = P[j - 1]; j--; }
      P[j] = x;
    }
    uint32_t w = 0;
    for (uint32_t r = 1; r < np; r++) {
      if (P[w].y >= P[r].x) P[w].y = max(P[w].y, P[r].y);
      else { w += 1; P[w] = P[r]; }
    }
    if (np) np = w + 1;
  }
  if (mine) {
    new_len[g] = len;
    n_pieces[g] = np;
  }
  {
    const unsigned long long sp = __ballot(fast && spilled);
    if (reach && sp && threadIdx.x == 0) atomicAdd(reach + VU_REACH_LANE_SPILL, (uint32_t)__popcll(sp));
  }
#ifdef IMPG_VU_CLOCKS
  VU_MARK(7);
  {
    const unsigned long long slow = 0ull, regp = __ballot(fast && spilled);
    const uint32_t nsum = wave_incl_scan(n), smax = 0u;
    const uint32_t ntot = (uint32_t)__builtin_amdgcn_readlane((int)nsum, 63);
    if (threadIdx.x == 0 && (blockIdx.x & 15u) == 0u) {
      unsigned long long *row = g_vu_clk[(blockIdx.x >> 4) % VU_CLK_ROWS];
      for (int i = 0; i < 7; i++) atomicAdd(&row[i], vu_t[i + 1] - vu_t[i]);
      atomicAdd(&row[8], 1ull);
      atomicAdd(&row[9], slow ? 1ull : 0ull);
      atomicAdd(&row[10], (unsigned long long)nmax);
      atomicAdd(&row[11], (unsigned long long)ntot);
      atomicAdd(&row[12], (unsigned long long)smax);
      atomicAdd(&row[13], regp ? 1ull : 0ull);
      if (slow) atomicAdd(&row[14], vu_t[3] - vu_t[2]);
    }
  }
#endif
  }
}
#pragma clang diagnostic pop
#ifdef IMPG_VU_CLOCKS
extern "C" void impg_gpu_debug_vu_clocks(unsigned long long *out) {
  static unsigned long long rows[VU_CLK_ROWS][16];
  (void)hipDeviceSynchronize();
  (void)hipMemcpyFromSymbol(rows, HIP_SYMBOL(g_vu_clk), sizeof(rows));
  for (int k = 0; k < 16; k++) { out[k] = 0; for (uint32_t r = 0; r < VU_CLK_ROWS; r++) out[k] += rows[r][k]; }
  memset(rows, 0, sizeof(rows));
  (void)hipMemcpyToSymbol(HIP_SYMBOL(g_vu_clk), rows, sizeof(rows));
}
#endif

template <class L> __device__ __forceinline__ void order_point(const L &) { __syncthreads(); }
struct ListSoA {
  int32_t *px, *py;
  __device__ __forceinline__ int32_t &x(uint32_t i) const { return px[i]; }
  __device__ __forceinline__ int32_t &y(uint32_t i) const { return py[i]; }
};
template <> __device__ __forceinline__ void order_point<ListSoA>(const ListSoA &) { __builtin_amdgcn_wave_barrier(); }
template <class L> __device__ __forceinline__ uint32_t wave_lower_bound(const L &R, uint32_t n, int32_t s) {
  uint32_t lo = 0, hi = n;
  const uint32_t lane = lane_id();
  while (hi - lo > 64u) {
    const uint32_t step = (hi - lo + 63u) >> 6;
    const uint32_t idx = lo + (lane + 1u) * step - 1u;
    const bool lt = idx < hi && R.x(idx) < s;
    const uint32_t c = (uint32_t)__popcll(__ballot(lt));
    const uint32_t nlo = lo + c * step;
    hi = min(hi, nlo + step);
    lo = nlo;
  }
  const uint32_t idx = lo + lane;
  return lo + (uint32_t)__popcll(__ballot(idx < hi && R.x(idx) < s));
}
template <class L> __device__ __forceinline__ void wave_shift_up(const L &R, uint32_t pos, uint32_t len) {
  const uint32_t lane = lane_id();
  for (uint32_t top = len; top > pos;) {
    const uint32_t base = top > pos + 64u ? top - 64u : pos;
    const uint32_t at = base + lane;
    const bool on = at < top;
    int32_t vx = 0, vy = 0;
    if (on) { vx = R.x(at); vy = R.y(at); }
    top = base;
    order_point(R);
    if (on) { R.x(at + 1) = vx; R.y(at + 1) = vy; }
    order_point(R);
  }
}
template <class L> __device__ __forceinline__ void wave_shift_down(const L &R, uint32_t from, uint32_t len, uint32_t k) {
  const uint32_t lane = lane_id();
  for (uint32_t base = from; base < len; base += 64u) {
    const uint32_t i = base + lane;
    int32_t vx = 0, vy = 0;
    if (i < len) { vx = R.x(i); vy = R.y(i); }
    order_point(R);
    if (i < len) { R.x(i - k) = vx; R.y(i - k) = vy; }
    order_point(R);
  }
}
__device__ __forceinline__ void sort_cx_lane(int2 &v, uint32_t partner) {
  int2 o;
// ... 540 lines not shown
  }
  keep[i] = covered ? 0u : 1u;
}
__global__ __launch_bounds__(256) void covered_compact_kernel(const unsigned long long *__restrict__ svals, const uint32_t *__restrict__ keep,
                                                              const uint32_t *__restrict__ kpos, uint32_t n_active,
                                                              unsigned long long *__restrict__ out) {
  const uint32_t i = blockIdx.x * 256u + threadIdx.x;
  if (i < n_active && keep[i]) out[kpos[i]] = svals[i];
}
__global__ __launch_bounds__(256) void covered_regroup_kernel(const uint32_t *__restrict__ kpos, uint32_t n_active, uint32_t n_kept,
                                                              uint32_t n_groups, uint32_t *__restrict__ gstart, uint32_t *__restrict__ glen,
                                                              uint32_t *__restrict__ cap, uint32_t *__restrict__ pcap) {
  const uint32_t g = blockIdx.x * 256u + threadIdx.x;
  if (g >= n_groups) return;
  const uint32_t st = gstart[g], n = glen[g], en = st + n;
  const uint32_t ns = kpos[st], ne = en < n_active ? kpos[en] : n_kept;
  const uint32_t olen = cap[g] - n;
  gstart[g] = ns;
  glen[g] = ne - ns;
  cap[g] = olen + (ne - ns);
  pcap[g] = olen + 2u * (ne - ns);
}

constexpr uint32_t BG_THREADS = 1024, BG_PER_THREAD = 4;
__global__ __launch_bounds__(BG_THREADS) void big_groups_kernel(const uint32_t *__restrict__ cap, const uint32_t *__restrict__ pcap,
                                                                uint32_t n_groups, uint32_t *__restrict__ big_list,
                                                                uint32_t *__restrict__ n_big) {
  __shared__ uint32_t cnt[4], base[4];
  if (threadIdx.x < 4u) cnt[threadIdx.x] = 0u;
  __syncthreads();
  uint32_t tier[BG_PER_THREAD], off[BG_PER_THREAD];
#pragma unroll
  for (uint32_t k = 0; k < BG_PER_THREAD; k++) {
    const uint32_t g = (blockIdx.x * BG_PER_THREAD + k) * BG_THREADS + threadIdx.x;
    const uint32_t c = g < n_groups ? cap[g] : 0u;
    uint32_t t = 0;
    if (c > VU_TINY_MAX) {
      if (c <= VU_MID_MAX) t = 1u;
      else {
        const uint32_t old_len = 2u * c - pcap[g];
        t = c + 64u <= VW_CAP_TINY ? 2u : (old_len + VW_SMALL_HEADROOM <= VW_CAP_SMALL - 64u ? 3u : 4u);
      }
    }
    tier[k] = t;
    off[k] = 0u;
    if (__ballot(t != 0u)) {
#pragma unroll
      for (uint32_t tt = 1; tt <= 4u; tt++) {
        const unsigned long long m = __ballot(t == tt);
        if (!m) continue;
        uint32_t o = 0;
        if (lane_id() == 0) o = atomicAdd(&cnt[tt - 1u], (uint32_t)__popcll(m));
        o = (uint32_t)__shfl((int)o, 0);
        if (t == tt) off[k] = o + (uint32_t)__popcll(m & lanemask_lt());
      }
    }
  }
  __syncthreads();
  if (threadIdx.x < 4u) {
    const uint32_t slot = threadIdx.x == 0u ? 6u : (threadIdx.x == 1u ? 2u : (threadIdx.x == 2u ? 0u : 1u));
    base[threadIdx.x] = cnt[threadIdx.x] ? atomicAdd(&n_big[slot], cnt[threadIdx.x]) : 0u;
  }
  __syncthreads();
#pragma unroll
  for (uint32_t k = 0; k < BG_PER_THREAD; k++) {
    const uint32_t g = (blockIdx.x * BG_PER_THREAD + k) * BG_THREADS + threadIdx.x;
    const uint32_t t = tier[k];
    if (!t) continue;
    const uint32_t pos = base[t - 1u] + off[k];
    if (t == 1u) big_list[2u * (size_t)n_groups + pos] = g;
    else if (t == 2u) big_list[(size_t)n_groups + pos] = g;
    else if (t == 3u) big_list[pos] = g;
    else big_list[n_groups - 1u - pos] = g;
  }
}

__global__ __launch_bounds__(256) void frontier_emit_kernel(const unsigned long long *__restrict__ gkey,
                                                            const uint32_t *__restrict__ poff,
                                                            const uint32_t *__restrict__ n_pieces,
                                                            const uint32_t *__restrict__ foff, uint32_t n_groups,
                                                            const int2 *__restrict__ pieces,
                                                            FrontierRec *__restrict__ out, const SegDesc *__restrict__ seg,
                                                            const int32_t *__restrict__ seq_len, uint32_t n_seq,
                                                            uint32_t *__restrict__ key, uint32_t *__restrict__ idx) {
  const uint32_t g = blockIdx.x * 256u + threadIdx.x;
  const bool in = g < n_groups;
  const unsigned long long k = in ? gkey[g] : 0ull;
  const uint32_t np = in ? n_pieces[g] : 0u;
  const uint32_t po = in ? poff[g] : 0u;
  const uint32_t fo = in ? foff[g] : 0xFFFFFFFFu;
  const uint32_t first = (uint32_t)__shfl((int)fo, 0);
  const unsigned long long live = __ballot(in);
  if (!live) return;
  const int last = 63 - __builtin_clzll(live);
  const uint32_t end = (uint32_t)__shfl((int)(fo + np), last);
  for (uint32_t o = first + lane_id(); o - lane_id() < end; o += 64u) {
    uint32_t j = 0;
#pragma unroll
    for (uint32_t st = 32u; st > 0u; st >>= 1) {
      const uint32_t f = (uint32_t)__shfl((int)fo, (int)(j + st));
      j += f <= o ? st : 0u;
    }
    const uint32_t fj = (uint32_t)__shfl((int)fo, (int)j), pj = (uint32_t)__shfl((int)po, (int)j);
    const uint32_t klo = (uint32_t)__shfl((int)(uint32_t)k, (int)j), khi = (uint32_t)__shfl((int)(uint32_t)(k >> 32), (int)j);
    if (o < end) {
      const int2 piece = pieces[pj + (o - fj)];
      FrontierRec f;
      f.target_id = klo;
      f.start = piece.x;
      f.end = piece.y;
      f.qidx = khi;
      out[o] = f;
      if (key) { key[o] = order_key(seg, seq_len, n_seq, klo, piece.x); if (idx) idx[o] = o; }
    }
  }
}

__global__ __launch_bounds__(256) void subset_filter_kernel(const FrontierRec *__restrict__ fr,
                                                            const uint32_t *__restrict__ pair_range, uint32_t n_pairs,
                                                            uint32_t *__restrict__ qid, const uint8_t *__restrict__ keep,
                                                            const impg_gpu_range_t *__restrict__ ranges) {
  const uint32_t p = blockIdx.x * 256u + threadIdx.x;
  if (p >= n_pairs) return;
  const uint32_t q = qid[p];
  if (q == HIT_NONE) return;
  if (keep[q]) return;
  if (q != ranges[fr[pair_range[p]].qidx].target_id) qid[p] = HIT_NONE;
}

__global__ __launch_bounds__(256) void mask_caps_kernel(const impg_gpu_range_t *__restrict__ ranges, uint32_t n,
                                                        const uint32_t *__restrict__ mask_off, uint32_t n_seq,
                                                        uint32_t *__restrict__ cap) {
  const uint32_t q = blockIdx.x * 256u + threadIdx.x;
  if (q >= n) return;
  const uint32_t t = ranges[q].target_id;
  cap[q] = (t < n_seq ? mask_off[t + 1] - mask_off[t] : 0u) + 1u;
}
__global__ __launch_bounds__(64) void visited_init_masked_kernel(const impg_gpu_range_t *__restrict__ ranges, uint32_t n,
                                                                 const int32_t *__restrict__ init_len, uint32_t n_seq,
                                                                 const uint32_t *__restrict__ mask_off,
                                                                 const int2 *__restrict__ mask_ranges,
                                                                 int32_t min_transitive_len, const uint32_t *__restrict__ loff,
                                                                 unsigned long long *__restrict__ keys,
                                                                 uint32_t *__restrict__ len_out, int2 *__restrict__ rng,
                                                                 int2 *__restrict__ pieces, uint32_t *__restrict__ n_self,
                                                                 uint32_t *__restrict__ n_front) {
  const uint32_t q = blockIdx.x * 64u + threadIdx.x;
  if (q >= n) return;
  const impg_gpu_range_t r = ranges[q];
  int32_t start = min(r.start, r.end), end = max(r.start, r.end);
  const bool known = r.target_id < n_seq;
  const int32_t sequence_length = known ? init_len[r.target_id] : 0;
  int2 *R = rng + loff[q];
  int2 *P = pieces + loff[q];
  uint32_t len = 0;
  if (known) {
    const uint32_t a = mask_off[r.target_id];
    len = mask_off[r.target_id + 1] - a;
    for (uint32_t i = 0; i < len; i++) R[i] = mask_ranges[a + i];
  }
  if (start < 0) start = 0;
  if (end > sequence_length) end = sequence_length;
  uint32_t np = 0, nf = 0;
  int32_t current = start;
  uint32_t i = lower_bound_start(R, len, start);
  if (i > 0 && R[i - 1].y > start) i -= 1;
  while (i < len && current < end) {
    const int2 rg = R[i];
    if (rg.x > end) break;
    if (current < rg.x) {
      P[np++] = make_int2(current, rg.x);
      nf += abs(rg.x - current) >= min_transitive_len;
    }
    current = max(current, rg.y);
    i += 1;
  }
  if (current < end) {
    P[np++] = make_int2(current, end);
    nf += abs(end - current) >= min_transitive_len;
  }
  const uint32_t pos = lower_bound_start(R, len, start);
  bool merge = true;
  uint32_t mfrom = 0;
  if (pos > 0 && R[pos - 1].y >= start) {
    R[pos - 1].y = max(R[pos - 1].y, end);
    mfrom = pos - 1;
  } else if (pos < len && end >= R[pos].x) {
    R[pos].x = min(start, R[pos].x);
    R[pos].y = max(end, R[pos].y);
    mfrom = pos;
  } else {
    for (uint32_t k = len; k > pos; k--) R[k] = R[k - 1];
    R[pos] = make_int2(start, end);
    len += 1;
    merge = false;
  }
// ... 757 lines not shown
  if (!n) return;
  prims::radix_sort_pairs(tmp, tmp_bytes, kin, kout, vin, vout, n, 0, end_bit, s);
}
bool seg_group_fits(uint32_t n_seq) { return n_seq <= SEG_MAX_SEQ; }
size_t seg_group_bins_bytes(uint32_t n_queries, uint32_t n_seq, uint32_t parts) {
  return (size_t)n_queries * parts * ((std::max(n_seq, 1u) + 63u) & ~63u) * 4;
}
uint32_t seg_group_parts(uint64_t n_hits, uint32_t n_queries, uint32_t n_seq, uint64_t largest_query) {
  if (!n_queries) return 1;
  const uint64_t per_query = std::max<uint64_t>(n_hits / n_queries, largest_query);
  if (per_query <= (largest_query ? SEG_BIG_QUERY : SEG_BIG_QUERY / 2)) return 1;
  const uint64_t parts = (per_query + SEG_SLICE_HITS - 1) / SEG_SLICE_HITS;
  if (parts > SEG_MAX_PARTS || (uint64_t)n_queries * parts >= (1ull << 31)) return 0;
  if (seg_group_bins_bytes(n_queries, n_seq, (uint32_t)parts) > (1ull << 30)) return 0;
  return (uint32_t)parts;
}
void launch_seg_bounds(const FrontierRec *fr, uint32_t n_fr, uint32_t n_queries, const uint32_t *pair_range, uint32_t n_pairs, uint32_t *run_start,
                       uint32_t *run_end, uint32_t *qfirst, uint32_t *qlast, uint32_t *unsorted, hipStream_t s, const uint32_t *off_perm,
                       const uint32_t *pair_off, const uint32_t *cnt) {
  IMPG_HIP(hipMemsetAsync(qfirst, 0, (size_t)n_queries * 4, s));
  IMPG_HIP(hipMemsetAsync(qlast, 0, (size_t)n_queries * 4, s));
  IMPG_HIP(hipMemsetAsync(unsorted, 0, 8, s));
  if (pair_off && cnt) {
    if (n_fr) run_bounds_by_offsets_kernel<<<cdiv(n_fr, 256), 256, 0, s>>>(off_perm, pair_off, cnt, n_fr, run_start, run_end);
  } else {
    IMPG_HIP(hipMemsetAsync(run_start, 0, (size_t)n_fr * 4, s));
    IMPG_HIP(hipMemsetAsync(run_end, 0, (size_t)n_fr * 4, s));
    if (n_pairs) run_bounds_kernel<<<cdiv(n_pairs, 256), 256, 0, s>>>(pair_range, n_pairs, run_start, run_end);
  }
  if (n_fr) query_bounds_kernel<<<cdiv(n_fr, 256), 256, 0, s>>>(fr, n_fr, n_queries, qfirst, qlast, unsorted);
}
void launch_seg_group(bool count_only, const FrontierRec *fr, const uint32_t *qfirst, const uint32_t *qlast, const uint32_t *run_start,
                      const uint32_t *run_end, HitArrays h, uint32_t n_queries, uint32_t n_seq, uint32_t *qact, const uint32_t *qdst, uint32_t *qgrp,
                      const uint32_t *gdst, uint32_t *gstart, unsigned long long *gkey, unsigned long long *svals, uint32_t *qbins, hipStream_t s,
                      uint32_t parts, uint32_t *qtot) {
  if (!n_queries) return;
  if (parts > 1u && (!qbins || !qtot)) throw Error{IMPG_E_INVALID, "internal: sliced segment grouping without its counters"};
  const uint32_t nb = (std::max(n_seq, 1u) + 63u) & ~63u;
  uint32_t nbits = 1;
  while ((1u << nbits) < n_seq) nbits++;
  const uint32_t grid = cdiv(n_queries * parts, SEG_WAVES);
  if (count_only)
    seg_group_kernel<true><<<grid, 64 * SEG_WAVES, SEG_WAVES * nb * 4, s>>>(fr, qfirst, qlast, run_start, run_end, h, n_queries, nb, nbits, qact, qdst, qgrp,
                                                                          gdst, gstart, gkey, svals, qbins, parts, qtot);
  else
    seg_group_kernel<false><<<grid, 64 * SEG_WAVES, SEG_WAVES * nb * 4, s>>>(fr, qfirst, qlast, run_start, run_end, h, n_queries, nb, nbits, qact, qdst, qgrp,
                                                                           gdst, gstart, gkey, svals, qbins, parts, qtot);
  if (count_only && parts > 1u) {
    IMPG_HIP(hipMemsetAsync(qact, 0, (size_t)n_queries * 4, s));
    IMPG_HIP(hipMemsetAsync(qgrp, 0, (size_t)n_queries * 4, s));
    seg_parts_scan_kernel<<<dim3(n_queries, cdiv(nb, 256u)), 256, 0, s>>>(qbins, nb, parts, qtot, qact, qgrp);
  }
}
uint32_t group_tiles(uint32_t n) { return (n + GROUP_TILE - 1u) / GROUP_TILE; }
void launch_group_count(const unsigned long long *skeys, uint32_t n, uint32_t *tile_heads, hipStream_t s) {
  if (n) group_count_kernel<<<group_tiles(n), 256, 0, s>>>(skeys, n, tile_heads);
}
void launch_group_fill(const unsigned long long *skeys, uint32_t n, const uint32_t *tile_base, uint32_t *gstart, unsigned long long *gkey, hipStream_t s) {
  if (n) group_fill_kernel<<<group_tiles(n), 256, 0, s>>>(skeys, n, tile_base, gstart, gkey);
}
void launch_group_heads(const unsigned long long *skeys, uint32_t n, uint32_t *head, hipStream_t s) {
  if (!n) return;
  group_heads_kernel<<<cdiv(n, 256), 256, 0, s>>>(skeys, n, head);
}
void launch_group_scatter(const unsigned long long *skeys, uint32_t n, const uint32_t *head, const uint32_t *gid,
                          uint32_t *gstart, unsigned long long *gkey, hipStream_t s) {
  if (!n) return;
  group_scatter_kernel<<<cdiv(n, 256), 256, 0, s>>>(skeys, n, head, gid, gstart, gkey);
}
void launch_table_qoff(const unsigned long long *keys, uint32_t n_groups, uint32_t n_queries, uint32_t *qoff, hipStream_t s) {
  table_qoff_kernel<<<cdiv((uint64_t)n_queries + 1, 256), 256, 0, s>>>(keys, n_groups, n_queries, qoff);
}
void launch_group_prepare(const VisitedTables &vt, const unsigned long long *gkey, const uint32_t *gstart,
                          uint32_t n_groups, uint32_t n_active, uint32_t *glen, const int2 **old_src,
                          uint32_t *cap, uint32_t *pcap, hipStream_t s) {
  if (!n_groups) return;
  group_prepare_kernel<<<cdiv(n_groups, 256), 256, 0, s>>>(vt, gkey, gstart, n_groups, n_active, glen, old_src, cap, pcap);
}
void launch_visited_update(const unsigned long long *svals, const int32_t *seq_len,
                           const unsigned long long *gkey, const uint32_t *gstart, const uint32_t *glen,
                           const int2 *const *old_src, const uint32_t *noff, const uint32_t *poff,
                           uint32_t n_groups, int32_t min_transitive_len, int32_t mdbr, int2 *new_ranges,
                           uint32_t *new_len, int2 *pieces, uint32_t *n_pieces, const uint32_t *cap, const uint32_t *pcap,
                           uint32_t *big_list, uint32_t *n_big, bool count_reach, hipStream_t s, const uint32_t *h_lists) {
  if (!n_groups) return;
  uint32_t *reach = count_reach ? n_big + VU_REACH_BASE : nullptr;
  const uint32_t n_small = h_lists[0], n_large = h_lists[1], n_tiny = h_lists[2], n_mid = h_lists[6];
  const unsigned long long *srcs = reinterpret_cast<const unsigned long long *>(old_src);
  visited_update_kernel<VU_LDS_CAP, false><<<cdiv(n_groups, 64), 64, 0, s>>>(svals, seq_len, gkey, gstart, glen, srcs, cap, noff, poff, n_groups,
                                                                             min_transitive_len, mdbr, new_ranges, new_len, pieces, n_pieces,
                                                                             nullptr, nullptr, reach);
  const uint32_t mid_blocks = std::min<uint32_t>(cdiv(n_mid, 64), 256u * std::min(32u, (160u * 1024u) / (VU_MID_CAP * 64u * 8u)));
  if (n_mid)
    visited_update_kernel<VU_MID_CAP, true><<<mid_blocks, 64, 0, s>>>(svals, seq_len, gkey, gstart, glen, srcs, cap, noff, poff, n_groups,
                                                                      min_transitive_len, mdbr, new_ranges, new_len, pieces, n_pieces,
                                                                      big_list + 2u * (size_t)n_groups, n_big + 6, reach);
  const uint32_t blocks = std::min<uint32_t>(n_small, 256u * std::min(32u, (160u * 1024u) / (VW_CAP_SMALL * 8u)));
  if (n_small)
    visited_update_wave_kernel<VW_CAP_SMALL><<<blocks, 64, 0, s>>>(
        svals, seq_len, gkey, gstart, glen, old_src, cap, noff, poff, big_list, n_big, n_big + 3, 0u, min_transitive_len, mdbr, new_ranges,
        new_len, pieces, n_pieces, reach);
  if (n_tiny)
    visited_update_wave_kernel<VW_CAP_TINY, true><<<std::min<uint32_t>(n_tiny, 256u * 32u), 64, 0, s>>>(
        svals, seq_len, gkey, gstart, glen, old_src, cap, noff, poff, big_list + n_groups, n_big + 2, n_big + 5, 0u, min_transitive_len, mdbr, new_ranges,
        new_len, pieces, n_pieces, reach);
  if (n_large)
    visited_update_wave_kernel<VW_CAP_LARGE><<<std::min<uint32_t>(n_large, 256u * 5u), 64, 0, s>>>(
        svals, seq_len, gkey, gstart, glen, old_src, cap, noff, poff, big_list, n_big + 1, n_big + 4, n_groups, min_transitive_len, mdbr,
        new_ranges, new_len, pieces, n_pieces, reach);
}
void launch_big_groups(const uint32_t *cap, const uint32_t *pcap, uint32_t n_groups, uint32_t *big_list, uint32_t *n_big, hipStream_t s) {
  if (!n_groups) return;
  (void)hipMemsetAsync(n_big, 0, VU_NBIG_WORDS * 4, s);
  big_groups_kernel<<<cdiv(n_groups, BG_THREADS * BG_PER_THREAD), BG_THREADS, 0, s>>>(cap, pcap, n_groups, big_list, n_big);
}
void launch_covered_flags(const unsigned long long *svals, const uint32_t *head, const uint32_t *gid,
                          const unsigned long long *gkey, const int2 *const *old_src, const uint32_t *cap, const uint32_t *glen,
                          const int32_t *seq_len, uint32_t n_active, uint32_t *keep, hipStream_t s) {
  if (n_active) covered_flags_kernel<<<cdiv(n_active, 256), 256, 0, s>>>(svals, head, gid, gkey, old_src, cap, glen, seq_len, n_active, keep);
}
void launch_covered_compact(const unsigned long long *svals, const uint32_t *keep, const uint32_t *kpos, uint32_t n_active,
                            unsigned long long *out, uint32_t n_kept, uint32_t n_groups, uint32_t *gstart, uint32_t *glen, uint32_t *cap,
                            uint32_t *pcap, hipStream_t s) {
  if (n_active) covered_compact_kernel<<<cdiv(n_active, 256), 256, 0, s>>>(svals, keep, kpos, n_active, out);
  if (n_groups) covered_regroup_kernel<<<cdiv(n_groups, 256), 256, 0, s>>>(kpos, n_active, n_kept, n_groups, gstart, glen, cap, pcap);
}
void launch_frontier_emit(const unsigned long long *gkey, const uint32_t *poff, const uint32_t *n_pieces,
                          const uint32_t *foff, uint32_t n_groups, const int2 *pieces, FrontierRec *out, hipStream_t s,
                          const DeviceIndexView *v, uint32_t *key, uint32_t *idx) {
  if (!n_groups) return;
  frontier_emit_kernel<<<cdiv(n_groups, 256), 256, 0, s>>>(gkey, poff, n_pieces, foff, n_groups, pieces, out, v ? v->seg : nullptr,
                                                           v ? v->seq_len : nullptr, v ? v->n_seq : 0u, v ? key : nullptr, v ? idx : nullptr);
}
void launch_subset_filter(const FrontierRec *fr, const uint32_t *pair_range, uint32_t n_pairs, uint32_t *qid,
                          const uint8_t *keep, const impg_gpu_range_t *ranges, hipStream_t s) {
  if (n_pairs) subset_filter_kernel<<<cdiv(n_pairs, 256), 256, 0, s>>>(fr, pair_range, n_pairs, qid, keep, ranges);
}
void launch_mask_caps(const impg_gpu_range_t *ranges, uint32_t n, const uint32_t *mask_off, uint32_t n_seq, uint32_t *cap,
                      hipStream_t s) {
  if (n) mask_caps_kernel<<<cdiv(n, 256), 256, 0, s>>>(ranges, n, mask_off, n_seq, cap);
}
void launch_visited_init_masked(const impg_gpu_range_t *ranges, uint32_t n, const int32_t *init_len, uint32_t n_seq,
                                const uint32_t *mask_off, const int2 *mask_ranges, int32_t min_transitive_len,
                                const uint32_t *loff, unsigned long long *keys, uint32_t *len, int2 *rng, int2 *pieces,
                                uint32_t *n_self, uint32_t *n_front, hipStream_t s) {
  if (n) visited_init_masked_kernel<<<cdiv(n, 64), 64, 0, s>>>(ranges, n, init_len, n_seq, mask_off, mask_ranges,
                                                                min_transitive_len, loff, keys, len, rng, pieces, n_self, n_front);
}
void launch_masked_self_emit(const impg_gpu_range_t *ranges, uint32_t n, const uint32_t *loff, const uint32_t *n_self,
                             const uint32_t *self_off, const uint32_t *front_off, int32_t min_transitive_len,
                             const int2 *pieces, FrontierRec *self_out, FrontierRec *frontier_out, hipStream_t s) {
  if (n) masked_self_emit_kernel<<<cdiv(n, 256), 256, 0, s>>>(ranges, n, loff, n_self, self_off, front_off, min_transitive_len,
                                                              pieces, self_out, frontier_out);
}
void launch_visited_init(const impg_gpu_range_t *ranges, uint32_t n, const int32_t *seq_len, uint32_t n_seq,
                         int32_t min_transitive_len, unsigned long long *keys, uint32_t *off, uint32_t *len, int2 *rng,
                         FrontierRec *self_iv, uint32_t *in_frontier, hipStream_t s) {
  if (!n) return;
  visited_init_kernel<<<cdiv(n, 256), 256, 0, s>>>(ranges, n, seq_len, n_seq, min_transitive_len, keys, off, len, rng, self_iv, in_frontier);
}
void launch_compact_frontier(const FrontierRec *in, const uint32_t *flag, const uint32_t *pos, uint32_t n,
                             FrontierRec *out, hipStream_t s) {
  if (!n) return;
  compact_frontier_kernel<<<cdiv(n, 256), 256, 0, s>>>(in, flag, pos, n, out);
}
void launch_ranges_to_frontier(const impg_gpu_range_t *ranges, uint32_t n, FrontierRec *out, uint32_t *bad, hipStream_t s) {
  if (!n) return;
  ranges_to_frontier_kernel<<<cdiv(n, 256), 256, 0, s>>>(ranges, n, out, bad);
}
void launch_frontier_to_stack(const FrontierRec *fr, uint32_t n, const uint32_t *pop_depth, bool use_depth,
                              unsigned long long *key, int32_t *st, int32_t *en, uint32_t *depth, hipStream_t s) {
  if (!n) return;
  frontier_to_stack_kernel<<<cdiv(n, 256), 256, 0, s>>>(fr, n, pop_depth, use_depth ? 1 : 0, key, st, en, depth);
}
void launch_dfs_pop_flags(const unsigned long long *key, const uint32_t *depth, uint32_t n, uint32_t max_depth,
                          bool pop_front, uint32_t *fr_flag, uint32_t *keep_flag, uint32_t *pop_depth, uint32_t *pop_sel, uint32_t n_queries,
                          hipStream_t s) {
  if (!n) return;
  IMPG_HIP(hipMemsetAsync(pop_sel, pop_front ? 0xFF : 0x00, (size_t)n_queries * 4, s));
  dfs_pop_select_kernel<<<cdiv(n, 256), 256, 0, s>>>(key, depth, n, max_depth, pop_front ? 1 : 0, pop_sel);
  dfs_pop_flags_kernel<<<cdiv(n, 256), 256, 0, s>>>(key, depth, n, pop_front ? 1 : 0, pop_sel, fr_flag, keep_flag, pop_depth);
}
void launch_sort5(const FrontierRec *fr, uint32_t n, const uint32_t *pair_off, uint32_t n_pairs, HitArrays h,
                  const uint32_t *pair_entry, const uint32_t *mrank, uint32_t *dest, hipStream_t s) {
  if (n && n_pairs) sort5_kernel<<<wave_grid(n), 256, 0, s>>>(fr, n, pair_off, n_pairs, h, pair_entry, mrank, dest);
}
void launch_permute_slots(const uint32_t *dest, uint32_t n_pairs, HitArrays in, HitArrays out, const uint32_t *pe_in,
                          uint32_t *pe_out, SliceArrays sin, SliceArrays sout, hipStream_t s) {
  if (n_pairs) permute_slots_kernel<<<cdiv(n_pairs, 256), 256, 0, s>>>(dest, n_pairs, in, out, pe_in, pe_out, sin, sout);
}
void launch_dfs_pop_scatter(const unsigned long long *key, const int32_t *st, const int32_t *en, const uint32_t *depth,
                            uint32_t n, const uint32_t *fr_flag, const uint32_t *fr_pos, const uint32_t *keep_flag,
                            const uint32_t *keep_pos, FrontierRec *fr_out, unsigned long long *key_out, int32_t *st_out,
                            int32_t *en_out, uint32_t *depth_out, hipStream_t s) {
  if (!n) return;
  dfs_pop_scatter_kernel<<<cdiv(n, 256), 256, 0, s>>>(key, st, en, depth, n, fr_flag, fr_pos, keep_flag, keep_pos, fr_out,
                                                     key_out, st_out, en_out, depth_out);
}
void launch_iota(uint32_t *v, uint32_t n, hipStream_t s) { if (n) iota_kernel<<<cdiv(n, 256), 256, 0, s>>>(v, n); }
void launch_gather_u32(const uint32_t *src, const uint32_t *idx, uint32_t n, uint32_t *dst, hipStream_t s) {
  if (n) gather_u32_kernel<<<cdiv(n, 256), 256, 0, s>>>(src, idx, n, dst);
}
void launch_gather_u64(const unsigned long long *src, const uint32_t *idx, uint32_t n, unsigned long long *dst, hipStream_t s) {
  if (n) gather_u64_kernel<<<cdiv(n, 256), 256, 0, s>>>(src, idx, n, dst);
}
void launch_run_heads(const unsigned long long *skeys, uint32_t n, uint32_t *head, hipStream_t s) {
  if (n) run_heads_kernel<<<cdiv(n, 256), 256, 0, s>>>(skeys, n, head);
}
void launch_run_starts(const uint32_t *head, const uint32_t *gid, uint32_t n, uint32_t *gstart, hipStream_t s) {
  if (n) run_starts_kernel<<<cdiv(n, 256), 256, 0, s>>>(head, gid, n, gstart);
}
void launch_dfs_merge(const uint32_t *gstart, uint32_t n_groups, uint32_t n, const uint32_t *perm, const int32_t *st,
                      const int32_t *en, const uint32_t *depth, int32_t *st_m, int32_t *en_m, uint32_t *depth_m,
                      uint32_t *cnt, hipStream_t s) {
  if (n_groups) dfs_merge_kernel<<<cdiv(n_groups, 64), 64, 0, s>>>(gstart, n_groups, n, perm, st, en, depth, st_m, en_m, depth_m, cnt);
// ... 279 lines not shown
```

### impg_amd/csrc/kernels.hpp

```cpp
#pragma once
#include <hip/hip_runtime.h>

#include <cstdint>

#include "impg_internal.hpp"

namespace impg {

struct FrontierRec {
  uint32_t target_id;
  int32_t start, end;
  uint32_t qidx;
};

struct HitArrays {
  uint32_t *qid;
  int4 *c;
};

struct SliceArrays {
  uint32_t *a;
  uint32_t *n;
  int32_t *off;
  int32_t *rem;
// ... 81 lines not shown
                        const uint32_t *pair_off, const uint4 *win, uint32_t *pair_range, uint32_t *pair_entry,
                        const uint32_t *perm, const uint32_t *offp, ProjList pl, const uint32_t *wide_n,
                        const uint32_t *wide_list, hipStream_t s, bool by_place = false, bool wide_only = false, WideEmit we = WideEmit{});
constexpr uint32_t ROUTE_WORLD_MAX = 1024;
void launch_route_keys(const FrontierRec *fr, uint32_t n, uint32_t world, const uint32_t *owner, uint32_t n_seq, uint32_t *key,
                       uint32_t *idx, unsigned long long *hist, hipStream_t s);
void launch_hits_pack(const FrontierRec *fr, const uint32_t *pair_range, uint32_t n_pairs, HitArrays h, const uint32_t *pair_entry,
                      const uint32_t *mrank, uint32_t words, void *out, hipStream_t s, const uint32_t *slice_n = nullptr);
void launch_hits_slice_n(const void *in, uint32_t n, uint32_t *cnt, hipStream_t s);
void launch_hits_unpack(const void *in, uint32_t n, uint32_t words, uint32_t n_front, const uint32_t *run_start, const uint32_t *off,
                        uint32_t *pair_range, HitArrays h, uint32_t *mslot, hipStream_t s, const uint32_t *slice_at = nullptr,
                        uint32_t *slice_pos = nullptr, uint32_t *slice_n = nullptr);
void launch_route_gather(const FrontierRec *fr, const uint32_t *perm, uint32_t n, FrontierRec *out, hipStream_t s);
void launch_route_gather_ranges(const FrontierRec *fr, const uint32_t *perm, uint32_t n, uint32_t range_base, FrontierRec *out, hipStream_t s);
void launch_partial_stats_add(const unsigned long long *in, uint32_t blocks, uint32_t n, unsigned long long *out, hipStream_t s);
void launch_frontier_gather(const FrontierRec *fr, const uint32_t *perm, uint32_t n, FrontierRec *out, hipStream_t s);
void launch_reorder_runs(const uint32_t *hits, uint32_t n, uint32_t words, uint32_t n_front, uint32_t *run_start,
                         uint32_t *run_len, uint32_t *err, hipStream_t s);
void launch_order_keys(const DeviceIndexView &v, const FrontierRec *fr, uint32_t n, uint32_t *key, uint32_t *idx, hipStream_t s,
                       const uint32_t *bounds = nullptr, uint32_t n_blocks = 0, uint32_t block_shift = 0);
void launch_scatter_u32(const uint32_t *in, const uint32_t *perm, uint32_t n, uint32_t *out, hipStream_t s);
enum ScanForm : int { SCAN_FORM_LOOKBACK = 0, SCAN_FORM_THREE_KERNEL = 1 };
int launch_exclusive_scan(const uint32_t *d_in, uint32_t *d_out, uint32_t n, unsigned long long *d_bsum,
                          unsigned long long *d_total, hipStream_t s);
size_t scan_scratch_bytes(uint32_t n);
void scan_tile_sizes(uint32_t *lookback_tile, uint32_t *three_kernel_tile);
enum ProjArm : int {
  PROJ_ARM_NONE = -1,
  PROJ_ARM_LANE = 0,
  PROJ_ARM_STAGED,
  PROJ_ARM_STAGED_ROWS,
  PROJ_ARM_ENTRIES_SLOTS,
  PROJ_ARM_ENTRIES_QS,
  PROJ_ARM_ENTRIES_ROWS,
  PROJ_ARM_ENTRIES_IDENT,
  PROJ_ARM_TP,
  PROJ_ARMS
};
static_assert(PROJ_ARMS == sizeof(impg_gpu_index::proj_stats) / sizeof(impg_gpu_index::proj_stats[0]), "one counter per arm");
enum UpdStat {
  UPD_LANE = 0, UPD_MID, UPD_WAVE_TINY, UPD_WAVE_SMALL, UPD_WAVE_LARGE,
  UPD_INPLACE,
  UPD_TILED_SORT,
  UPD_LANE_SPILL,
  UPD_STATS
};
static_assert(UPD_STATS == sizeof(impg_gpu_index::upd_stats) / sizeof(impg_gpu_index::upd_stats[0]), "one counter per path");
int launch_project(const DeviceIndexView &v, const FrontierRec *fr, const uint32_t *pair_range,
                   const uint32_t *pair_entry, uint32_t n_pairs, bool transitive, HitArrays h,
                   unsigned long long *accepted, uint32_t *err_flag, double min_identity, const SliceArrays *slices,
                   ProjList pl, hipStream_t s, const uint32_t *n_pairs_dev = nullptr, bool regroup = false,
                   const WindowLists *wl = nullptr);
constexpr uint32_t SMALL_HEADER_BYTES = 64;
void launch_small_scan(const uint32_t *cnt, uint32_t n, uint32_t *off, uint32_t *total, hipStream_t s);
void launch_small_pack(const FrontierRec *fr, const uint32_t *pair_range, const uint32_t *n_pairs_dev, uint32_t pairs_bound, HitArrays h,
                       const uint32_t *err_flag, const unsigned long long *accepted, void *hdr, impg_gpu_interval_t *rows,
                       uint32_t *row_range, hipStream_t s);
void launch_slice_counts(HitArrays h, SliceArrays sl, uint32_t n_pairs, uint32_t *cnt, hipStream_t s);
void launch_slice_write(const DeviceIndexView &v, const uint32_t *pair_entry, HitArrays h, SliceArrays sl, uint32_t n_pairs,
                        const uint32_t *off, uint32_t *out, hipStream_t s);
void launch_hit_stats(const FrontierRec *fr, uint32_t n_fr, const uint32_t *pair_range, uint32_t n_pairs, HitArrays h,
                      int32_t min_output_length, bool skip_same_target, unsigned long long *rstat, unsigned long long *count,
                      unsigned long long *cksum, hipStream_t s, uint32_t stride = 1 );
void launch_sort5(const FrontierRec *fr, uint32_t n, const uint32_t *pair_off, uint32_t n_pairs, HitArrays h,
                  const uint32_t *pair_entry, const uint32_t *mrank, uint32_t *dest, hipStream_t s);
void launch_permute_slots(const uint32_t *dest, uint32_t n_pairs, HitArrays in, HitArrays out, const uint32_t *pe_in,
                          uint32_t *pe_out, SliceArrays sin, SliceArrays sout, hipStream_t s);
void launch_update_keys(const FrontierRec *fr, const uint32_t *pair_range, uint32_t n_pairs, HitArrays h,
                        unsigned long long *keys, unsigned long long *vals, unsigned long long *n_active, hipStream_t s);
size_t sort_pairs_scratch_bytes(uint32_t n);
void launch_sort_pairs(void *tmp, size_t tmp_bytes, const unsigned long long *kin, unsigned long long *kout,
                       const uint32_t *vin, uint32_t *vout, uint32_t n, unsigned end_bit, hipStream_t s);
uint32_t group_tiles(uint32_t n);
void launch_group_count(const unsigned long long *skeys, uint32_t n, uint32_t *tile_heads, hipStream_t s);
void launch_group_fill(const unsigned long long *skeys, uint32_t n, const uint32_t *tile_base, uint32_t *gstart, unsigned long long *gkey, hipStream_t s);
void launch_group_heads(const unsigned long long *skeys, uint32_t n, uint32_t *head, hipStream_t s);
void launch_group_scatter(const unsigned long long *skeys, uint32_t n, const uint32_t *head, const uint32_t *gid,
                          uint32_t *gstart, unsigned long long *gkey, hipStream_t s);
void launch_table_qoff(const unsigned long long *keys, uint32_t n_groups, uint32_t n_queries, uint32_t *qoff, hipStream_t s);
void launch_group_prepare(const VisitedTables &vt, const unsigned long long *gkey, const uint32_t *gstart,
                          uint32_t n_groups, uint32_t n_active, uint32_t *glen, const int2 **old_src,
                          uint32_t *cap, uint32_t *pcap, hipStream_t s);
constexpr uint32_t VU_NBIG_WORDS = 12, VU_REACH_BASE = 8, VU_REACH_INPLACE = 0, VU_REACH_TILED_SORT = 1, VU_REACH_LANE_SPILL = 2;
void launch_visited_update(const unsigned long long *svals, const int32_t *seq_len,
                           const unsigned long long *gkey, const uint32_t *gstart, const uint32_t *glen,
                           const int2 *const *old_src, const uint32_t *noff, const uint32_t *poff,
                           uint32_t n_groups, int32_t min_transitive_len, int32_t mdbr, int2 *new_ranges,
                           uint32_t *new_len, int2 *pieces, uint32_t *n_pieces, const uint32_t *cap, const uint32_t *pcap,
                           uint32_t *big_list, uint32_t *n_big, bool count_reach, hipStream_t s, const uint32_t *h_lists);
constexpr uint32_t VU_LIST_WORDS = 7;
void launch_big_groups(const uint32_t *cap, const uint32_t *pcap, uint32_t n_groups, uint32_t *big_list, uint32_t *n_big, hipStream_t s);
void launch_covered_flags(const unsigned long long *svals, const uint32_t *head, const uint32_t *gid,
                          const unsigned long long *gkey, const int2 *const *old_src, const uint32_t *cap, const uint32_t *glen,
                          const int32_t *seq_len, uint32_t n_active, uint32_t *keep, hipStream_t s);
void launch_covered_compact(const unsigned long long *svals, const uint32_t *keep, const uint32_t *kpos, uint32_t n_active,
                            unsigned long long *out, uint32_t n_kept, uint32_t n_groups, uint32_t *gstart, uint32_t *glen, uint32_t *cap,
                            uint32_t *pcap, hipStream_t s);
void launch_frontier_emit(const unsigned long long *gkey, const uint32_t *poff, const uint32_t *n_pieces,
                          const uint32_t *foff, uint32_t n_groups, const int2 *pieces, FrontierRec *out, hipStream_t s,
                          const DeviceIndexView *v = nullptr, uint32_t *key = nullptr, uint32_t *idx = nullptr);
void launch_subset_filter(const FrontierRec *fr, const uint32_t *pair_range, uint32_t n_pairs, uint32_t *qid,
                          const uint8_t *keep, const impg_gpu_range_t *ranges, hipStream_t s);
void launch_mask_caps(const impg_gpu_range_t *ranges, uint32_t n, const uint32_t *mask_off, uint32_t n_seq, uint32_t *cap,
                      hipStream_t s);
void launch_visited_init_masked(const impg_gpu_range_t *ranges, uint32_t n, const int32_t *init_len, uint32_t n_seq,
                                const uint32_t *mask_off, const int2 *mask_ranges, int32_t min_transitive_len,
                                const uint32_t *loff, unsigned long long *keys, uint32_t *len, int2 *rng, int2 *pieces,
                                uint32_t *n_self, uint32_t *n_front, hipStream_t s);
void launch_masked_self_emit(const impg_gpu_range_t *ranges, uint32_t n, const uint32_t *loff, const uint32_t *n_self,
                             const uint32_t *self_off, const uint32_t *front_off, int32_t min_transitive_len,
                             const int2 *pieces, FrontierRec *self_out, FrontierRec *frontier_out, hipStream_t s);
void launch_visited_init(const impg_gpu_range_t *ranges, uint32_t n, const int32_t *seq_len, uint32_t n_seq,
                         int32_t min_transitive_len, unsigned long long *keys, uint32_t *off, uint32_t *len, int2 *rng,
                         FrontierRec *self_iv, uint32_t *in_frontier, hipStream_t s);
void launch_compact_frontier(const FrontierRec *in, const uint32_t *flag, const uint32_t *pos, uint32_t n,
                             FrontierRec *out, hipStream_t s);
void launch_ranges_to_frontier(const impg_gpu_range_t *ranges, uint32_t n, FrontierRec *out, uint32_t *bad, hipStream_t s);

void launch_frontier_to_stack(const FrontierRec *fr, uint32_t n, const uint32_t *pop_depth, bool use_depth,
                              unsigned long long *key, int32_t *st, int32_t *en, uint32_t *depth, hipStream_t s);
void launch_dfs_pop_flags(const unsigned long long *key, const uint32_t *depth, uint32_t n, uint32_t max_depth,
                          bool pop_front, uint32_t *fr_flag, uint32_t *keep_flag, uint32_t *pop_depth, uint32_t *pop_sel ,
                          uint32_t n_queries, hipStream_t s);
void launch_dfs_pop_scatter(const unsigned long long *key, const int32_t *st, const int32_t *en, const uint32_t *depth,
                            uint32_t n, const uint32_t *fr_flag, const uint32_t *fr_pos, const uint32_t *keep_flag,
                            const uint32_t *keep_pos, FrontierRec *fr_out, unsigned long long *key_out, int32_t *st_out,
                            int32_t *en_out, uint32_t *depth_out, hipStream_t s);
void launch_iota(uint32_t *v, uint32_t n, hipStream_t s);
void launch_gather_u32(const uint32_t *src, const uint32_t *idx, uint32_t n, uint32_t *dst, hipStream_t s);
void launch_gather_u64(const unsigned long long *src, const uint32_t *idx, uint32_t n, unsigned long long *dst, hipStream_t s);
void launch_run_heads(const unsigned long long *skeys, uint32_t n, uint32_t *head, hipStream_t s);
void launch_run_starts(const uint32_t *head, const uint32_t *gid, uint32_t n, uint32_t *gstart, hipStream_t s);
void launch_dfs_merge(const uint32_t *gstart, uint32_t n_groups, uint32_t n, const uint32_t *perm, const int32_t *st,
                      const int32_t *en, const uint32_t *depth, int32_t *st_m, int32_t *en_m, uint32_t *depth_m,
                      uint32_t *cnt, hipStream_t s);
void launch_dfs_compact(const uint32_t *gstart, const uint32_t *cnt, const uint32_t *off, uint32_t n_groups,
                        const unsigned long long *skeys, const int32_t *st_m, const int32_t *en_m, const uint32_t *depth_m,
                        unsigned long long *key_out, int32_t *st_out, int32_t *en_out, uint32_t *depth_out, hipStream_t s);
size_t sort_u32_scratch_bytes(uint32_t n);
void launch_sort_u32(void *tmp, size_t tmp_bytes, const uint32_t *kin, uint32_t *kout, const uint32_t *vin, uint32_t *vout,
                     uint32_t n, hipStream_t s, unsigned begin_bit = 0, unsigned end_bit = 32);
size_t order_sort_scratch_bytes(uint32_t n);
void launch_order_sort(uint32_t *keys, uint32_t *key_tmp, uint32_t *perm_out, uint32_t *perm_tmp, uint32_t n, unsigned end_bit, void *scratch,
                       hipStream_t s);
#ifdef IMPG_OS_CLOCKS
void order_sort_clocks(unsigned long long *out, bool reset);
#endif
size_t sort_u64v_scratch_bytes(uint32_t n);
void launch_sort_u64v(void *tmp, size_t tmp_bytes, const unsigned long long *kin, unsigned long long *kout,
                      const unsigned long long *vin, unsigned long long *vout, uint32_t n, hipStream_t s, unsigned end_bit = 64,
                      unsigned begin_bit = 0);
void launch_compact_fill(const unsigned long long *keys, uint32_t n, uint32_t table, unsigned long long *key_out,
                         unsigned long long *src_out, hipStream_t s);
void launch_compact_last(const unsigned long long *skeys, uint32_t n, uint32_t *flag, hipStream_t s);
void launch_compact_select(const VisitedTables &vt, const unsigned long long *skeys, const unsigned long long *ssrc, uint32_t n,
                           const uint32_t *flag, const uint32_t *pos, unsigned long long *key_out,
                           unsigned long long *src_out, uint32_t *len_out, hipStream_t s);
void launch_compact_copy(const VisitedTables &vt, const unsigned long long *src, const uint32_t *off, const uint32_t *len,
                         uint32_t n, int2 *ranges_out, hipStream_t s);

bool seg_group_fits(uint32_t n_seq);
void launch_seg_bounds(const FrontierRec *fr, uint32_t n_fr, uint32_t n_queries, const uint32_t *pair_range, uint32_t n_pairs, uint32_t *run_start,
                       uint32_t *run_end, uint32_t *qfirst, uint32_t *qlast, uint32_t *unsorted, hipStream_t s, const uint32_t *off_perm = nullptr,
                       const uint32_t *pair_off = nullptr, const uint32_t *cnt = nullptr);
void launch_seg_group(bool count_only, const FrontierRec *fr, const uint32_t *qfirst, const uint32_t *qlast, const uint32_t *run_start,
                      const uint32_t *run_end, HitArrays h, uint32_t n_queries, uint32_t n_seq, uint32_t *qact, const uint32_t *qdst, uint32_t *qgrp,
                      const uint32_t *gdst, uint32_t *gstart, unsigned long long *gkey, unsigned long long *svals, uint32_t *qbins, hipStream_t s,
                      uint32_t parts = 1, uint32_t *qtot = nullptr);
size_t seg_group_bins_bytes(uint32_t n_queries, uint32_t n_seq, uint32_t parts = 1);
uint32_t seg_group_parts(uint64_t n_hits, uint32_t n_queries, uint32_t n_seq, uint64_t largest_query = 0);

struct WalkArgs {
  DeviceIndexView v;
  const impg_gpu_range_t *ranges;
  uint32_t n_queries;
  int dfs;
  uint32_t max_depth;
  int32_t min_transitive_len, mdbr, min_output_length;
  double min_identity;
  const uint8_t *subset_keep;
  unsigned long long *count, *cksum;
  unsigned long long *accepted;
  uint32_t *err_flag;
// ... 37 lines not shown
```

### impg_amd/csrc/options.hpp

```cpp
#pragma once
#include <cstddef>
#include <cstdint>
#include <cstdlib>

namespace impg {

struct Options {
  int64_t pair_budget = 1ll << 28;
  int64_t chunk_ranges = 0;
  int64_t locality_min = 4096;
  int64_t device_rows_pool_bytes = 160ll << 30;
  int64_t fuse_final_level = 1;
  int64_t regroup_entries = 1;
  int64_t walk_kernel = 1;
  int64_t segment_groups = 1;
  int64_t segment_parts = 0;
  int64_t walk_members = 0;
  int64_t filter_covered = 0;
  int64_t update_stats = 0;
  int64_t lookup_stats = 0;
  int64_t wide_emit_cap = 4096;
  int64_t wide_emit_bins = 1024;
  int64_t lookup_coop = 1;
  int64_t lookup_coop_span = 256;
  int64_t place_offsets_blocks = 1;
  int64_t approximate_cigar = 0;
  int64_t free_slot_order = 1;
  int64_t debug_fail_owner = 0, debug_fail_home = 0;
  int64_t bed_text_piece_bytes = 256ll << 20;
  int64_t bedpe_group_log2 = 2;
  int64_t paf_group_log2 = 2;
  int64_t sequence_store_packed = 0;
  int64_t sequence_ingest_piece_bytes = 64ll << 20;
  int64_t lane_schedule = 0;
};

struct OptionRow {
  const char *key;
  int64_t lo, hi;
  int64_t Options::*member;
  bool flag;
  bool to_ranks;
  const char *refusal;
};
constexpr OptionRow OPTION_TABLE[] = {
    {"pair_budget", 1024, 0xFFFFFFEFll, &Options::pair_budget, false, true, "pair_budget out of range"},
    {"chunk_ranges", 0, (1ll << 31) - 1, &Options::chunk_ranges, false, true, "chunk_ranges out of range"},
    {"locality_min", 0, (1ll << 31) - 1, &Options::locality_min, false, true, "locality_min out of range"},
    {"device_rows_pool_bytes", 0, INT64_MAX, &Options::device_rows_pool_bytes, false, true, "device_rows_pool_bytes must not be negative"},
    {"fuse_final_level", INT64_MIN, INT64_MAX, &Options::fuse_final_level, true, true, ""},
    {"regroup_entries", INT64_MIN, INT64_MAX, &Options::regroup_entries, true, false, ""},
    {"walk_kernel", 0, 2, &Options::walk_kernel, false, false, "walk_kernel is 0, 1 or 2"},
    {"segment_groups", INT64_MIN, INT64_MAX, &Options::segment_groups, true, false, ""},
    {"segment_parts", 0, 4096, &Options::segment_parts, false, false, "segment_parts is 0 .. 4096"},
    {"walk_members", 0, 64, &Options::walk_members, false, false, "walk_members is 0 .. 64"},
    {"filter_covered", 0, 2, &Options::filter_covered, false, false, "filter_covered is 0, 1 or 2"},
    {"update_stats", INT64_MIN, INT64_MAX, &Options::update_stats, true, false, ""},
    {"lookup_stats", INT64_MIN, INT64_MAX, &Options::lookup_stats, true, false, ""},
    {"wide_emit_cap", 64, 4096, &Options::wide_emit_cap, false, false, "wide_emit_cap is 64 .. 4096"},
    {"wide_emit_bins", 2, 1024, &Options::wide_emit_bins, false, false, "wide_emit_bins is 2 .. 1024"},
    {"lookup_coop", INT64_MIN, INT64_MAX, &Options::lookup_coop, true, false, ""},
    {"lookup_coop_span", 4, 256, &Options::lookup_coop_span, false, false, "lookup_coop_span is 4 .. 256"},
    {"place_offsets_blocks", INT64_MIN, INT64_MAX, &Options::place_offsets_blocks, true, false, ""},
    {"approximate_cigar", 0, 1, &Options::approximate_cigar, false, true, "approximate_cigar is 0 or 1"},
    {"free_slot_order", INT64_MIN, INT64_MAX, &Options::free_slot_order, true, false, ""},
    {"debug_fail_owner", 0, 0xFFFFFFFFll, &Options::debug_fail_owner, false, true, "debug_fail_* out of range"},
    {"debug_fail_home", 0, 0xFFFFFFFFll, &Options::debug_fail_home, false, true, "debug_fail_* out of range"},
    {"lane_schedule", 0, INT64_MAX, &Options::lane_schedule, false, true, "lane_schedule out of range"},
    {"bed_text_piece_bytes", 64, 1ll << 40, &Options::bed_text_piece_bytes, false, false, "bed_text_piece_bytes is 64 .. 2^40"},
    {"bedpe_group_log2", 2, 6, &Options::bedpe_group_log2, false, false, "bedpe_group_log2 is 2 .. 6"},
    {"paf_group_log2", 2, 6, &Options::paf_group_log2, false, false, "paf_group_log2 is 2 .. 6"},
    {"sequence_store_packed", 0, 2, &Options::sequence_store_packed, false, false, "sequence_store_packed is 0, 1 or 2"},
    {"sequence_ingest_piece_bytes", 16, 1ll << 32, &Options::sequence_ingest_piece_bytes, false, false, "sequence_ingest_piece_bytes is 16 .. 2^32, a multiple of 16"},
    {"prewarm_result_bytes", 0, INT64_MAX, nullptr, false, false, "prewarm_result_bytes is a size"},
    {"prewarm_walk", 0, 2, nullptr, false, false, "prewarm_walk is 0, 1 or 2"},
};
constexpr size_t N_OPTIONS = sizeof(OPTION_TABLE) / sizeof(OPTION_TABLE[0]);

constexpr const OptionRow *option_row(const char *key) {
  for (const OptionRow &r : OPTION_TABLE)
    if (__builtin_strcmp(r.key, key) == 0) return &r;
  return nullptr;
}
inline bool option_store(Options &o, const OptionRow &r, int64_t value) {
  if (value < r.lo || value > r.hi) return false;
  if (r.member) o.*r.member = r.flag ? (int64_t)(value != 0) : value;
  return true;
}
inline void options_to_ranks(const Options &from, Options &rank) {
  for (const OptionRow &r : OPTION_TABLE)
    if (r.to_ranks) rank.*r.member = from.*r.member;
}

struct BuildSwitches {
  bool prefix_lines;
  bool identity_lines;
  bool host_build;
  bool timing;
  uint64_t batch_ops;
};
constexpr uint64_t BUILD_BATCH_OPS = 64ull << 20;
inline BuildSwitches build_switches() {
  const char *pfx = getenv("IMPG_PREFIX_LINES"), *idl = getenv("IMPG_IDENTITY_LINES"), *bat = getenv("IMPG_BUILD_BATCH_OPS");
  const unsigned long long b = bat ? strtoull(bat, nullptr, 10) : 0ull;
  return BuildSwitches{!(pfx && atoi(pfx) == 0), idl && atoi(idl) == 1, getenv("IMPG_BUILD_HOST") != nullptr, getenv("IMPG_BUILD_TIMING") != nullptr,
                       b ? (uint64_t)b : BUILD_BATCH_OPS};
}

}
```

Measured before the change: 82.50 billion.

## Emit next frontier directly from visited-update kernel on the final hop

When the next level is the last one and output order does not matter, the visited-update kernel now writes merged frontier records straight from LDS into the next-frontier buffer. It reserves output space with a wave/block-level scan plus an atomic cursor. This skips writing new visited ranges and lengths and skips registering a new visited table, since no later level will consult it. Spilled or wave-tier groups still go through the piece-based frontier_emit path, which appends after the cursor. It also adds a 2-wave block variant for the emitting kernel, plus a debug getenv print and a counter.

New measurement: 82.85 billion (median of 6 runs). Within noise of the previous version (+0.4%).

```diff
diff --git a/impg_amd/csrc/capi.cpp b/impg_amd/csrc/capi.cpp
--- a/impg_amd/csrc/capi.cpp
+++ b/impg_amd/csrc/capi.cpp
@@ -40,6 +40,7 @@
   e->seg_stats = ix.seg_stats;
   e->proj_stats = ix.proj_stats;
   e->place_block_levels = &ix.place_block_levels;
+  e->emit_levels = &ix.emit_levels;
   e->upd_stats = ix.upd_stats;
   e->dfs_stats = ix.dfs_stats;
   e->lk_stats = ix.lk_stats;
@@ -646,7 +647,7 @@
     CTR("project_staged_rows_levels", proj_stats[PROJ_ARM_STAGED_ROWS]), CTR("project_entries_slots_levels", proj_stats[PROJ_ARM_ENTRIES_SLOTS]),
     CTR("project_entries_qs_levels", proj_stats[PROJ_ARM_ENTRIES_QS]), CTR("project_entries_rows_levels", proj_stats[PROJ_ARM_ENTRIES_ROWS]),
     CTR("project_entries_ident_levels", proj_stats[PROJ_ARM_ENTRIES_IDENT]), CTR("project_tp_levels", proj_stats[PROJ_ARM_TP]),
-    CTR("place_offsets_block_levels", place_block_levels),
+    CTR("place_offsets_block_levels", place_block_levels), CTR("update_emit_levels", emit_levels),
     CTR("update_lane_groups", upd_stats[UPD_LANE]), CTR("update_mid_groups", upd_stats[UPD_MID]), CTR("update_wave_tiny_groups", upd_stats[UPD_WAVE_TINY]),
     CTR("update_wave_small_groups", upd_stats[UPD_WAVE_SMALL]), CTR("update_wave_large_groups", upd_stats[UPD_WAVE_LARGE]),
     CTR("update_inplace_groups", upd_stats[UPD_INPLACE]), CTR("update_tiled_sort_groups", upd_stats[UPD_TILED_SORT]),
diff --git a/impg_amd/csrc/engine.cpp b/impg_amd/csrc/engine.cpp
--- a/impg_amd/csrc/engine.cpp
+++ b/impg_amd/csrc/engine.cpp
@@ -596,7 +596,7 @@
 }
 
 uint32_t Engine::update(const DeviceIndexView &v, const FrontierRec *fr, LevelBufs &L, uint32_t n_queries,
-                        const impg_gpu_params_t &p, DevBuf &next_frontier) {
+                        const impg_gpu_params_t &p, DevBuf &next_frontier, bool last_any_order) {
   hipEvent_t e0 = event(), e1 = event();
   IMPG_HIP(hipEventRecord(e0, stream));
   const uint32_t P = L.n_pairs;
@@ -750,18 +750,37 @@
             VU_LIST_WORDS);
       if (cap_total >= 0xFFFFFFF0ull || pcap_total >= 0xFFFFFFF0ull)
         { if (split_ok) throw SplitBatch{}; throw Error{IMPG_E_UNSUPPORTED, "visited sets exceed 2^32 ranges"}; }
-      vt->ranges.reserve(std::max<size_t>(cap_total * 8, 256));
-      vt->len.reserve((size_t)n_groups * 4);
+      const bool emit_path = last_any_order && opt.update_emit_frontier && !remote && !masked && !multi && !store_cigar && pcap_total < (1ull << 31);
+      if (getenv("IMPG_DEBUG_GROUPS"))
+        fprintf(stderr, "[groups] cap_total=%llu pcap_total=%llu emit=%d\n", (unsigned long long)cap_total, (unsigned long long)pcap_total, (int)emit_path);
+      const bool wave_tiers = h_lists[0] || h_lists[1] || h_lists[2];
+      if (!emit_path || wave_tiers) {
+        vt->ranges.reserve(std::max<size_t>(cap_total * 8, 256));
+        vt->len.reserve((size_t)n_groups * 4);
+      }
       pieces.reserve(std::max<size_t>(pcap_total * 8, 256));
       n_pieces.reserve((size_t)n_groups * 4);
       foff.reserve((size_t)n_groups * 4);
+      FrontierEmit fe{nullptr, nullptr, nullptr, d_nbig + VU_EMIT_CURSOR, v.seg, v.n_seq};
+      const bool emit_keys = emit_path && opt.locality_min && pcap_total >= (uint64_t)opt.locality_min;
+      if (emit_path) {
+        next_frontier.reserve(std::max<size_t>((size_t)pcap_total * sizeof(FrontierRec), 256));
+        fe.out = next_frontier.as<FrontierRec>();
+        if (emit_keys) {
+          lo_key.reserve(std::max<size_t>((size_t)pcap_total * 4, 256)); lo_idx.reserve(std::max<size_t>((size_t)pcap_total * 4, 256));
+          fe.key = lo_key.as<uint32_t>();
+          fe.idx = lib_sort_selected() ? lo_idx.as<uint32_t>() : nullptr;
+        }
+      }
       launch_visited_update(replay_vals, masked ? mask_touch_len.as<int32_t>() : v.seq_len, vt->keys.as<unsigned long long>(),
                             gstart.as<uint32_t>(), glen.as<uint32_t>(), old_src.as<const int2 *>(),
                             vt->off.as<uint32_t>(), poff.as<uint32_t>(), n_groups, p.min_transitive_len,
                             p.min_distance_between_ranges, vt->ranges.as<int2>(), vt->len.as<uint32_t>(),
                             pieces.as<int2>(), n_pieces.as<uint32_t>(), cap.as<uint32_t>(), pcap.as<uint32_t>(), big_list.as<uint32_t>(),
-                            d_nbig, opt.update_stats && upd_stats, stream, h_lists);
-      uint64_t nn = scan(n_pieces.as<uint32_t>(), foff.as<uint32_t>(), n_groups);
+                            d_nbig, opt.update_stats && upd_stats, stream, h_lists, emit_path ? &fe : nullptr);
+      uint32_t n_emitted = 0;
+      uint64_t nn = scan(n_pieces.as<uint32_t>(), foff.as<uint32_t>(), n_groups, emit_path ? fe.cursor : nullptr, &n_emitted, emit_path ? 1u : 0u);
+      nn += n_emitted;
       if (opt.update_stats && upd_stats && n_groups) {
         IMPG_HIP(hipMemcpyAsync(h_counters, counters.as<uint64_t>() + 8, VU_NBIG_WORDS * 4, hipMemcpyDeviceToHost, stream));
         IMPG_HIP(hipStreamSynchronize(stream));
@@ -777,18 +796,27 @@
       }
       if (nn >= 0xFFFFFFF0ull) { if (split_ok) throw SplitBatch{}; throw Error{IMPG_E_UNSUPPORTED, "frontier exceeds 2^32 ranges"}; }
       n_next = (uint32_t)nn;
-      next_frontier.reserve(std::max<size_t>((size_t)n_next * sizeof(FrontierRec), 256));
-      const bool keys_too = !remote && opt.locality_min && n_next >= opt.locality_min;
-      if (keys_too) { lo_key.reserve((size_t)n_next * 4); lo_idx.reserve((size_t)n_next * 4); }
-      launch_frontier_emit(vt->keys.as<unsigned long long>(), poff.as<uint32_t>(), n_pieces.as<uint32_t>(),
-                           foff.as<uint32_t>(), n_groups, pieces.as<int2>(), next_frontier.as<FrontierRec>(), stream,
-                           keys_too ? &v : nullptr, lo_key.as<uint32_t>(), lib_sort_selected() ? lo_idx.as<uint32_t>() : nullptr);
-      keys_for = keys_too ? next_frontier.p : nullptr;
-      keys_n = n_next;
-      vt->n_groups = n_groups;
-      index_table(*vt);
-      tables.push_back(std::move(vt));
-      if (tables.size() + 2 >= (size_t)MAX_VISITED_TABLES) compact_tables();
+      if (emit_path) {
+        launch_frontier_emit(vt->keys.as<unsigned long long>(), poff.as<uint32_t>(), n_pieces.as<uint32_t>(),
+                             foff.as<uint32_t>(), n_groups, pieces.as<int2>(), fe.out, stream,
+                             emit_keys ? &v : nullptr, fe.key, fe.idx, fe.cursor);
+        keys_for = emit_keys && n_next >= opt.locality_min ? next_frontier.p : nullptr;
+        keys_n = n_next;
+        if (emit_levels) (*emit_levels)++;
+      } else {
+        next_frontier.reserve(std::max<size_t>((size_t)n_next * sizeof(FrontierRec), 256));
+        const bool keys_too = !remote && opt.locality_min && n_next >= opt.locality_min;
+        if (keys_too) { lo_key.reserve((size_t)n_next * 4); lo_idx.reserve((size_t)n_next * 4); }
+        launch_frontier_emit(vt->keys.as<unsigned long long>(), poff.as<uint32_t>(), n_pieces.as<uint32_t>(),
+                             foff.as<uint32_t>(), n_groups, pieces.as<int2>(), next_frontier.as<FrontierRec>(), stream,
+                             keys_too ? &v : nullptr, lo_key.as<uint32_t>(), lib_sort_selected() ? lo_idx.as<uint32_t>() : nullptr);
+        keys_for = keys_too ? next_frontier.p : nullptr;
+        keys_n = n_next;
+        vt->n_groups = n_groups;
+        index_table(*vt);
+        tables.push_back(std::move(vt));
+        if (tables.size() + 2 >= (size_t)MAX_VISITED_TABLES) compact_tables();
+      }
     }
   }
   IMPG_HIP(hipEventRecord(e1, stream));
@@ -991,7 +1019,9 @@
                          transitive ? p.min_output_length : -1, false, rstat.as<unsigned long long>(), d_count, d_cksum, stream);
       }
       if (st) st->levels += 1;
-      if (!last) n_next = update(v, cur->as<FrontierRec>(), *L, n, p, *nxt);
+      const bool next_last = p.max_depth > 0 && depth + 2 >= p.max_depth;
+      if (!last) n_next = update(v, cur->as<FrontierRec>(), *L, n, p, *nxt,
+                                 next_last && free_slot_order && (!keep || spec.keep_any_order) && !ordered_rows);
       if (keep && !owners_keep) {
         if (L->placed) {
         } else if (last_range_places && !remote) {
diff --git a/impg_amd/csrc/engine.hpp b/impg_amd/csrc/engine.hpp
--- a/impg_amd/csrc/engine.hpp
+++ b/impg_amd/csrc/engine.hpp
@@ -143,7 +143,8 @@
   HopResult hop(const DeviceIndexView &v, const FrontierRec *fr, uint32_t n_fr, bool transitive, LevelBufs &L,
                 impg_gpu_stats_t *st, bool need_hits, bool need_rows, bool alive);
   uint32_t update(const DeviceIndexView &v, const FrontierRec *fr, LevelBufs &L, uint32_t n_queries,
-                  const impg_gpu_params_t &p, DevBuf &next_frontier);
+                  const impg_gpu_params_t &p, DevBuf &next_frontier,
+                  bool last_any_order = false);
   VisitedTables tables_view() const;
   void compact_tables();
   DevBuf dk_a, dk_b, ds_a, ds_b, de_a, de_b, dd_a, dd_b, d_flag2, d_pos2, d_popdepth, d_popsel, d_perm, d_perm2, d_k32, d_k32b,
@@ -192,6 +193,7 @@
   std::atomic<uint64_t> *upd_stats = nullptr;
   std::atomic<uint64_t> *dfs_stats = nullptr;
   std::atomic<uint64_t> *place_block_levels = nullptr;
+  std::atomic<uint64_t> *emit_levels = nullptr;
   void count_arm(int arm) { if (proj_stats && arm >= 0 && arm < PROJ_ARMS) proj_stats[arm]++; }
   uint32_t walk_group_size(const impg_gpu_index &ix, uint32_t n, const impg_gpu_params_t &p) const;
   char *small_in = nullptr;
diff --git a/impg_amd/csrc/impg_internal.hpp b/impg_amd/csrc/impg_internal.hpp
--- a/impg_amd/csrc/impg_internal.hpp
+++ b/impg_amd/csrc/impg_internal.hpp
@@ -378,6 +378,7 @@
   mutable std::atomic<uint64_t> seg_stats[3] = {};
   mutable std::atomic<uint64_t> proj_stats[8] = {};
   mutable std::atomic<uint64_t> place_block_levels{0};
+  mutable std::atomic<uint64_t> emit_levels{0};
   mutable std::atomic<uint64_t> upd_stats[8] = {};
   mutable std::atomic<uint64_t> lk_stats[8] = {};
   mutable std::atomic<uint64_t> refine_stats[5] = {};
diff --git a/impg_amd/csrc/kernels.hip b/impg_amd/csrc/kernels.hip
--- a/impg_amd/csrc/kernels.hip
+++ b/impg_amd/csrc/kernels.hip
@@ -3059,8 +3059,19 @@
 #endif
 #pragma clang diagnostic push
 #pragma clang diagnostic ignored "-Wpass-failed"
-template <uint32_t CAP, bool LISTED>
-__global__ __launch_bounds__(64) __attribute__((amdgpu_waves_per_eu(IMPG_VU_WAVES, IMPG_VU_WAVES)))
+struct UpdateEmit {
+  FrontierRec *out;
+  uint32_t *key, *idx;
+  uint32_t *cursor;
+  const SegDesc *seg;
+  uint32_t n_seq;
+};
+#ifndef IMPG_VU_EMIT_WAVES
+#define IMPG_VU_EMIT_WAVES 2
+#endif
+constexpr uint32_t vu_block_waves(bool listed, bool emit) { return emit && !listed ? IMPG_VU_EMIT_WAVES : 1u; }
+template <uint32_t CAP, bool LISTED, bool EMIT>
+__global__ __launch_bounds__(64 * vu_block_waves(LISTED, EMIT)) __attribute__((amdgpu_waves_per_eu(IMPG_VU_WAVES, IMPG_VU_WAVES)))
 void visited_update_kernel(const unsigned long long *__restrict__ svals,
                                                             const int32_t *__restrict__ seq_len,
                                                             const unsigned long long *__restrict__ gkey,
@@ -3074,10 +3085,12 @@
                                                             int2 *__restrict__ new_ranges, uint32_t *__restrict__ new_len,
                                                             int2 *__restrict__ pieces, uint32_t *__restrict__ n_pieces,
                                                             const uint32_t *__restrict__ list, const uint32_t *__restrict__ n_list,
-                                                            uint32_t *__restrict__ reach) {
-  __shared__ int32_t lds_x[CAP * 64], lds_y[CAP * 64];
+                                                            uint32_t *__restrict__ reach, const UpdateEmit em) {
+  constexpr uint32_t WV = vu_block_waves(LISTED, EMIT);
+  __shared__ int32_t lds_x[CAP * 64 * WV], lds_y[CAP * 64 * WV];
+  const uint32_t lane = WV == 1u ? threadIdx.x : (threadIdx.x & 63u), col0 = WV == 1u ? threadIdx.x : (threadIdx.x >> 6) * CAP * 64u + lane;
   const uint32_t n_items = LISTED ? *n_list : n_groups;
-  for (uint32_t item0 = blockIdx.x * 64u; item0 < n_items; item0 += gridDim.x * 64u) {
+  for (uint32_t item0 = blockIdx.x * 64u * WV; item0 < n_items; item0 += gridDim.x * 64u * WV) {
   const uint32_t item = item0 + threadIdx.x;
 #ifdef IMPG_VU_CLOCKS
   unsigned long long vu_t[8];
@@ -3107,7 +3120,7 @@
   uint32_t len = olen, np = 0;
   VU_MARK(3);
   const bool fast = mine;
-  const ListInLds A{lds_x + threadIdx.x, lds_y + threadIdx.x};
+  const ListInLds A{lds_x + col0, lds_y + col0};
   if (fast) {
     if (olen > 0) { A.x(0) = s0.x; A.y(0) = s0.y; }
     if (olen > 1) { A.x(1) = s1.x; A.y(1) = s1.y; }
@@ -3154,7 +3167,7 @@
     h0 = q0; h1 = q1; h2 = q2; h3 = q3;
   }
   VU_MARK(5);
-  if (fast) for (uint32_t i = 0; i < len; i++) R[i] = make_int2(A.x(i), A.y(i));
+  if (!EMIT && fast) for (uint32_t i = 0; i < len; i++) R[i] = make_int2(A.x(i), A.y(i));
   VU_MARK(6);
   if (fast && !spilled) {
     const uint32_t T = CAP - 1u;
@@ -3170,13 +3183,16 @@
       for (uint32_t r = 1; r < np; r++) {
         const int32_t rx = A.x(T - r), ry = A.y(T - r);
         if (cy >= rx) cy = max(cy, ry);
-        else { P[w] = make_int2(cx, cy); w += 1; cx = rx; cy = ry; }
+        else {
+          if (EMIT) { A.x(T - w) = cx; A.y(T - w) = cy; } else P[w] = make_int2(cx, cy);
+          w += 1; cx = rx; cy = ry;
+        }
       }
-      P[w] = make_int2(cx, cy);
+      if (EMIT) { A.x(T - w) = cx; A.y(T - w) = cy; } else P[w] = make_int2(cx, cy);
       np = w + 1;
     }
   } else if (mine && np > 1 && np <= CAP) {
-    const ListInLds S{lds_x + threadIdx.x, lds_y + threadIdx.x};
+    const ListInLds S{lds_x + col0, lds_y + col0};
     for (uint32_t i = 0; i < np; i += 4) {
       const uint32_t l = np - 1u;
       const int2 r0 = P[i], r1 = P[min(i + 1u, l)], r2 = P[min(i + 2u, l)], r3 = P[min(i + 3u, l)];
@@ -3214,13 +3230,61 @@
     }
     if (np) np = w + 1;
   }
-  if (mine) {
+  if (EMIT) {
+    const uint32_t ne = fast && !spilled ? np : 0u;
+    const uint32_t inc = wave_incl_scan(ne), fo = inc - ne;
+    const uint32_t tot = (uint32_t)__builtin_amdgcn_readlane((int)inc, 63);
+    uint32_t base = 0;
+    if (WV == 1u) {
+      if (tot && lane == 0u) base = atomicAdd(em.cursor, tot);
+    } else {
+      __shared__ uint32_t wave_tot[WV], block_base;
+      const uint32_t w = threadIdx.x >> 6;
+      if (lane == 0u) wave_tot[w] = tot;
+      __syncthreads();
+      if (threadIdx.x == 0u) {
+        uint32_t sum = 0;
+        for (uint32_t k = 0; k < WV; k++) sum += wave_tot[k];
+        block_base = sum ? atomicAdd(em.cursor, sum) : 0u;
+      }
+      __syncthreads();
+      base = block_base;
+      for (uint32_t k = 0; k < w; k++) base += wave_tot[k];
+    }
+    base = (uint32_t)__builtin_amdgcn_readfirstlane((int)base);
+    if (tot) {
+      const int32_t *wx = lds_x + (col0 - lane), *wy = lds_y + (col0 - lane);
+      __builtin_amdgcn_wave_barrier();
+      for (uint32_t o = lane; o - lane < tot; o += 64u) {
+        uint32_t j = 0;
+#pragma unroll
+        for (uint32_t sh = 32u; sh > 0u; sh >>= 1) {
+          const uint32_t f = (uint32_t)__shfl((int)fo, (int)(j + sh));
+          j += f <= o ? sh : 0u;
+        }
+        const uint32_t fj = (uint32_t)__shfl((int)fo, (int)j);
+        const uint32_t klo = (uint32_t)__shfl((int)(uint32_t)key, (int)j), khi = (uint32_t)__shfl((int)(uint32_t)(key >> 32), (int)j);
+        if (o < tot) {
+          const uint32_t e = (CAP - 1u - (o - fj)) * 64u + j;
+          FrontierRec f;
+          f.target_id = klo;
+          f.start = wx[e];
+          f.end = wy[e];
+          f.qidx = khi;
+          em.out[base + o] = f;
+          if (em.key) { em.key[base + o] = order_key(em.seg, seq_len, em.n_seq, klo, f.start); if (em.idx) em.idx[base + o] = base + o; }
+        }
+      }
+      __builtin_amdgcn_wave_barrier();
+    }
+    if (mine) n_pieces[g] = fast && !spilled ? 0u : np;
+  } else if (mine) {
     new_len[g] = len;
     n_pieces[g] = np;
   }
   {
     const unsigned long long sp = __ballot(fast && spilled);
-    if (reach && sp && threadIdx.x == 0) atomicAdd(reach + VU_REACH_LANE_SPILL, (uint32_t)__popcll(sp));
+    if (reach && sp && lane == 0u) atomicAdd(reach + VU_REACH_LANE_SPILL, (uint32_t)__popcll(sp));
   }
 #ifdef IMPG_VU_CLOCKS
   VU_MARK(7);
@@ -3927,7 +3991,8 @@
                                                             const int2 *__restrict__ pieces,
                                                             FrontierRec *__restrict__ out, const SegDesc *__restrict__ seg,
                                                             const int32_t *__restrict__ seq_len, uint32_t n_seq,
-                                                            uint32_t *__restrict__ key, uint32_t *__restrict__ idx) {
+                                                            uint32_t *__restrict__ key, uint32_t *__restrict__ idx,
+                                                            const uint32_t *__restrict__ cursor) {
   const uint32_t g = blockIdx.x * 256u + threadIdx.x;
   const bool in = g < n_groups;
   const unsigned long long k = in ? gkey[g] : 0ull;
@@ -3939,6 +4004,8 @@
   if (!live) return;
   const int last = 63 - __builtin_clzll(live);
   const uint32_t end = (uint32_t)__shfl((int)(fo + np), last);
+  if (end == first) return;
+  const uint32_t cb = cursor ? *cursor : 0u;
   for (uint32_t o = first + lane_id(); o - lane_id() < end; o += 64u) {
     uint32_t j = 0;
 #pragma unroll
@@ -3955,8 +4022,8 @@
       f.start = piece.x;
       f.end = piece.y;
       f.qidx = khi;
-      out[o] = f;
-      if (key) { key[o] = order_key(seg, seq_len, n_seq, klo, piece.x); if (idx) idx[o] = o; }
+      out[cb + o] = f;
+      if (key) { key[cb + o] = order_key(seg, seq_len, n_seq, klo, piece.x); if (idx) idx[cb + o] = cb + o; }
     }
   }
 }
@@ -4880,19 +4947,30 @@
                            const int2 *const *old_src, const uint32_t *noff, const uint32_t *poff,
                            uint32_t n_groups, int32_t min_transitive_len, int32_t mdbr, int2 *new_ranges,
                            uint32_t *new_len, int2 *pieces, uint32_t *n_pieces, const uint32_t *cap, const uint32_t *pcap,
-                           uint32_t *big_list, uint32_t *n_big, bool count_reach, hipStream_t s, const uint32_t *h_lists) {
+                           uint32_t *big_list, uint32_t *n_big, bool count_reach, hipStream_t s, const uint32_t *h_lists,
+                           const FrontierEmit *fe) {
   if (!n_groups) return;
   uint32_t *reach = count_reach ? n_big + VU_REACH_BASE : nullptr;
+  const UpdateEmit em = fe ? UpdateEmit{fe->out, fe->key, fe->idx, fe->cursor, fe->seg, fe->n_seq} : UpdateEmit{nullptr, nullptr, nullptr, nullptr, nullptr, 0u};
   const uint32_t n_small = h_lists[0], n_large = h_lists[1], n_tiny = h_lists[2], n_mid = h_lists[6];
   const unsigned long long *srcs = reinterpret_cast<const unsigned long long *>(old_src);
-  visited_update_kernel<VU_LDS_CAP, false><<<cdiv(n_groups, 64), 64, 0, s>>>(svals, seq_len, gkey, gstart, glen, srcs, cap, noff, poff, n_groups,
+  if (fe)
+    visited_update_kernel<VU_LDS_CAP, false, true><<<cdiv(n_groups, 64u * vu_block_waves(false, true)), 64u * vu_block_waves(false, true), 0, s>>>(svals, seq_len, gkey, gstart, glen, srcs, cap, noff, poff, n_groups,
+                                                                                     min_transitive_len, mdbr, new_ranges, new_len, pieces, n_pieces,
+                                                                                     nullptr, nullptr, reach, em);
+  else
+    visited_update_kernel<VU_LDS_CAP, false, false><<<cdiv(n_groups, 64), 64, 0, s>>>(svals, seq_len, gkey, gstart, glen, srcs, cap, noff, poff, n_groups,
+                                                                                      min_transitive_len, mdbr, new_ranges, new_len, pieces, n_pieces,
+                                                                                      nullptr, nullptr, reach, em);
+  const uint32_t mid_blocks = std::min<uint32_t>(cdiv(n_mid, 64), 256u * std::min(32u, (160u * 1024u) / (VU_MID_CAP * 64u * 8u)));
+  if (n_mid && fe)
+    visited_update_kernel<VU_MID_CAP, true, true><<<mid_blocks, 64, 0, s>>>(svals, seq_len, gkey, gstart, glen, srcs, cap, noff, poff, n_groups,
+                                                                            min_transitive_len, mdbr, new_ranges, new_len, pieces, n_pieces,
+                                                                            big_list + 2u * (size_t)n_groups, n_big + 6, reach, em);
+  else if (n_mid)
+    visited_update_kernel<VU_MID_CAP, true, false><<<mid_blocks, 64, 0, s>>>(svals, seq_len, gkey, gstart, glen, srcs, cap, noff, poff, n_groups,
                                                                              min_transitive_len, mdbr, new_ranges, new_len, pieces, n_pieces,
-                                                                             nullptr, nullptr, reach);
-  const uint32_t mid_blocks = std::min<uint32_t>(cdiv(n_mid, 64), 256u * std::min(32u, (160u * 1024u) / (VU_MID_CAP * 64u * 8u)));
-  if (n_mid)
-    visited_update_kernel<VU_MID_CAP, true><<<mid_blocks, 64, 0, s>>>(svals, seq_len, gkey, gstart, glen, srcs, cap, noff, poff, n_groups,
-                                                                      min_transitive_len, mdbr, new_ranges, new_len, pieces, n_pieces,
-                                                                      big_list + 2u * (size_t)n_groups, n_big + 6, reach);
+                                                                             big_list + 2u * (size_t)n_groups, n_big + 6, reach, em);
   const uint32_t blocks = std::min<uint32_t>(n_small, 256u * std::min(32u, (160u * 1024u) / (VW_CAP_SMALL * 8u)));
   if (n_small)
     visited_update_wave_kernel<VW_CAP_SMALL><<<blocks, 64, 0, s>>>(
@@ -4925,10 +5003,10 @@
 }
 void launch_frontier_emit(const unsigned long long *gkey, const uint32_t *poff, const uint32_t *n_pieces,
                           const uint32_t *foff, uint32_t n_groups, const int2 *pieces, FrontierRec *out, hipStream_t s,
-                          const DeviceIndexView *v, uint32_t *key, uint32_t *idx) {
+                          const DeviceIndexView *v, uint32_t *key, uint32_t *idx, const uint32_t *cursor) {
   if (!n_groups) return;
   frontier_emit_kernel<<<cdiv(n_groups, 256), 256, 0, s>>>(gkey, poff, n_pieces, foff, n_groups, pieces, out, v ? v->seg : nullptr,
-                                                           v ? v->seq_len : nullptr, v ? v->n_seq : 0u, v ? key : nullptr, v ? idx : nullptr);
+                                                           v ? v->seq_len : nullptr, v ? v->n_seq : 0u, v ? key : nullptr, v ? idx : nullptr, cursor);
 }
 void launch_subset_filter(const FrontierRec *fr, const uint32_t *pair_range, uint32_t n_pairs, uint32_t *qid,
                           const uint8_t *keep, const impg_gpu_range_t *ranges, hipStream_t s) {
diff --git a/impg_amd/csrc/kernels.hpp b/impg_amd/csrc/kernels.hpp
--- a/impg_amd/csrc/kernels.hpp
+++ b/impg_amd/csrc/kernels.hpp
@@ -187,12 +187,21 @@
                           uint32_t n_groups, uint32_t n_active, uint32_t *glen, const int2 **old_src,
                           uint32_t *cap, uint32_t *pcap, hipStream_t s);
 constexpr uint32_t VU_NBIG_WORDS = 12, VU_REACH_BASE = 8, VU_REACH_INPLACE = 0, VU_REACH_TILED_SORT = 1, VU_REACH_LANE_SPILL = 2;
+constexpr uint32_t VU_EMIT_CURSOR = 7;
+struct FrontierEmit {
+  FrontierRec *out;
+  uint32_t *key, *idx;
+  uint32_t *cursor;
+  const SegDesc *seg;
+  uint32_t n_seq;
+};
 void launch_visited_update(const unsigned long long *svals, const int32_t *seq_len,
                            const unsigned long long *gkey, const uint32_t *gstart, const uint32_t *glen,
                            const int2 *const *old_src, const uint32_t *noff, const uint32_t *poff,
                            uint32_t n_groups, int32_t min_transitive_len, int32_t mdbr, int2 *new_ranges,
                            uint32_t *new_len, int2 *pieces, uint32_t *n_pieces, const uint32_t *cap, const uint32_t *pcap,
-                           uint32_t *big_list, uint32_t *n_big, bool count_reach, hipStream_t s, const uint32_t *h_lists);
+                           uint32_t *big_list, uint32_t *n_big, bool count_reach, hipStream_t s, const uint32_t *h_lists,
+                           const FrontierEmit *emit = nullptr);
 constexpr uint32_t VU_LIST_WORDS = 7;
 void launch_big_groups(const uint32_t *cap, const uint32_t *pcap, uint32_t n_groups, uint32_t *big_list, uint32_t *n_big, hipStream_t s);
 void launch_covered_flags(const unsigned long long *svals, const uint32_t *head, const uint32_t *gid,
@@ -203,7 +212,8 @@
                             uint32_t *pcap, hipStream_t s);
 void launch_frontier_emit(const unsigned long long *gkey, const uint32_t *poff, const uint32_t *n_pieces,
                           const uint32_t *foff, uint32_t n_groups, const int2 *pieces, FrontierRec *out, hipStream_t s,
-                          const DeviceIndexView *v = nullptr, uint32_t *key = nullptr, uint32_t *idx = nullptr);
+                          const DeviceIndexView *v = nullptr, uint32_t *key = nullptr, uint32_t *idx = nullptr,
+                          const uint32_t *cursor = nullptr);
 void launch_subset_filter(const FrontierRec *fr, const uint32_t *pair_range, uint32_t n_pairs, uint32_t *qid,
                           const uint8_t *keep, const impg_gpu_range_t *ranges, hipStream_t s);
 void launch_mask_caps(const impg_gpu_range_t *ranges, uint32_t n, const uint32_t *mask_off, uint32_t n_seq, uint32_t *cap,
diff --git a/impg_amd/csrc/options.hpp b/impg_amd/csrc/options.hpp
--- a/impg_amd/csrc/options.hpp
+++ b/impg_amd/csrc/options.hpp
@@ -24,6 +24,7 @@
   int64_t lookup_coop = 1;
   int64_t lookup_coop_span = 256;
   int64_t place_offsets_blocks = 1;
+  int64_t update_emit_frontier = 1;
   int64_t approximate_cigar = 0;
   int64_t free_slot_order = 1;
   int64_t debug_fail_owner = 0, debug_fail_home = 0;
@@ -62,6 +63,7 @@
     {"lookup_coop", INT64_MIN, INT64_MAX, &Options::lookup_coop, true, false, ""},
     {"lookup_coop_span", 4, 256, &Options::lookup_coop_span, false, false, "lookup_coop_span is 4 .. 256"},
     {"place_offsets_blocks", INT64_MIN, INT64_MAX, &Options::place_offsets_blocks, true, false, ""},
+    {"update_emit_frontier", INT64_MIN, INT64_MAX, &Options::update_emit_frontier, true, true, ""},
     {"approximate_cigar", 0, 1, &Options::approximate_cigar, false, true, "approximate_cigar is 0 or 1"},
     {"free_slot_order", INT64_MIN, INT64_MAX, &Options::free_slot_order, true, false, ""},
     {"debug_fail_owner", 0, 0xFFFFFFFFll, &Options::debug_fail_owner, false, true, "debug_fail_* out of range"},
```
